# Nemo1999/Joint-TensoRF

Hardware: NVIDIA B200
Metric: rays/sec fwd+bwd (300^3 VM, 4096-ray batch) (higher is better)
Workload: dtype f32 (basis/shading GEMMs on tcgen05: bf16 operands, f32 accumulate)

## Files before the change

### include/jt_vm.h

```cpp
#ifndef JT_VM_H_
#define JT_VM_H_

#include <stdint.h>

#ifdef __cplusplus
extern "C" {
#endif

#ifndef __CUDA_RUNTIME_H__
typedef struct CUstream_st* cudaStream_t;
#endif

const char* jt_strerror(int code);
int jt_version(void);
long long jt_launch_count(void);

int jt_sample_ray_dense(const float* rays_o, const float* rays_d, const float* aux, int ndc, int n_rays,
                        int n_samples, const float* h_geom, const uint32_t* mask_bits, const int* h_mask_dims,
                        const float* h_mask_geom, float* pts, float* z, uint8_t* valid, cudaStream_t stream);

int jt_march_compact(const float* rays_o, const float* rays_d, const float* aux, int ndc, int n_rays,
                     int n_samples, const float* h_geom, const uint32_t* mask_bits, const int* h_mask_dims,
                     const float* h_mask_geom, int* ray_cnt, int* ray_off, int* sidx, float* samp, float* dist,
                     cudaStream_t stream);

int jt_exclusive_scan(const int* cnt, int* off, int n, cudaStream_t stream);

int jt_vm_gather_fwd(int app, const void* const* h_factors, const int* h_dims, const float* samp,
                     const int* slot, const int* n_dev, int n_max, float* out, cudaStream_t stream);

int jt_vm_gather_bwd(int app, const void* const* h_factors, void* const* h_factor_grads, const int* h_dims,
                     const float* samp, const int* slot, const int* n_dev, int n_max, const float* gin,
                     float* dsamp, int accumulate, cudaStream_t stream);

int jt_vm_scatter_rays(int app, const void* const* h_factors, void* const* h_factor_grads, const int* h_dims,
                       const float* samp, const int* slot, const int* sidx, const int* n_dev, int n_max,
                       const void* gin, int gin_bf16, int n_samples, const float* h_inv, float* d_o, float* d_d,
                       int max_ctas, int plane_mask, cudaStream_t stream);
int jt_ray_init(const float* rays_d, const float* dnorm, int n_rays, float* d_o, float* d_d, cudaStream_t stream);

int jt_gemm_nt(const float* X, int ldx, const float* W, int ldw, int w_kn, const float* bias, float* Y, int ldy,
               const float* mask, int ldm, const int* m_dev, int m_max, int N, int K, int act,
               cudaStream_t stream);
int jt_gemm_tn(const float* dY, int ldy, const float* X, int ldx, const int* m_dev, int m_max, int N, int K,
               float* dW, int ldw, float* db, cudaStream_t stream);
int jt_pe_encode(int bwd, int app_dim, int fea_pe, int view_pe, int mode, float fea_progress,
                 float view_progress, int n_samples, int normalize_dir, const float* feat, int ldf,
                 const int* aidx, const int* sidx, const float* rays_d, const int* n_dev, int n_max, float* out,
                 int ldo, float* out2, int ldo2, const float* din, int ldi, cudaStream_t stream);
int jt_sh_shade(int bwd, const float* feat, int ldf, const int* aidx, const int* sidx, const float* rays_d,
                int n_samples, int normalize_dir, const int* n_dev, int n_max, float* rgb, const float* dout,
                float* dfeat, int ldd, cudaStream_t stream);

int jt_tc_selftest(int mode, const float* A, int lda, const float* B, int ldb, float* D, int K, int N, int Ma,
                   cudaStream_t stream);
long long jt_head_tc_stage_bytes(int n_max);
int jt_head_fwd_tc(int split, const float* comps, const int* aidx, const int* sidx, const float* rays_d,
                   int n_samples, int normalize_dir, const float* Wb, const float* W1, const float* b1,
                   const float* W2, const float* b2, const float* W3, const float* b3, const int* n_dev, int n_max,
                   float fea_progress, float view_progress, float* rgb, float* feat_out, void* stage,
                   cudaStream_t stream);
int jt_app_basis_fwd_tc(int split, const void* const* h_factors, const int* h_dims, const float* samp,
                        const int* aidx, const int* sidx, const float* rays_d, int n_samples, int normalize_dir,
                        const float* Wb, const int* n_dev, int n_max, float* featdir, void* stage,
                        cudaStream_t stream);
int jt_head_mlp_fwd_tc(int split, const float* featdir, const float* W1, const float* b1, const float* W2,
                       const float* b2, const float* W3, const float* b3, const int* n_dev, int n_max,
                       float fea_progress, float view_progress, float* rgb, void* stage, cudaStream_t stream);
int jt_head_bwd_tc(const float* dout, const float* feat, int ldf, const float* Wb, const float* W1, const float* W2,
                   const float* W3, const int* n_dev, int n_max, float fea_progress, void* dcomps, int dcomps_bf16, void* stage,
                   float* gWb, float* gW1, float* gb1, float* gW2, float* gb2, float* gW3, float* gb3,
                   cudaStream_t stream);
int jt_app_basis_sh_fwd_tc(int split, const void* const* h_factors, const int* h_dims, const float* samp,
                           const int* aidx, const int* sidx, const float* rays_d, int n_samples, int normalize_dir,
                           const float* Wb, const int* n_dev, int n_max, float* featdir, float* rgb, void* stage,
                           cudaStream_t stream);
int jt_sh_bwd_tc(const float* dout, const float* featdir, int ldf, const float* Wb, const int* n_dev, int n_max,
                 void* dcomps, int dcomps_bf16, void* stage, float* gWb, cudaStream_t stream);

int jt_alpha_fwd(const int* ray_off, int n_rays, const float* sigfeat, const float* dist, const float* samp,
                 float density_shift, int act, float distance_scale, float thres, float* weight, float* trans,
                 float* acc, float* wz, int* app_cnt, int* app_off, int* aidx, int* app_of, int app_cap,
                 int* app_used, cudaStream_t stream);
int jt_composite_fwd(const int* app_off, int n_rays, const int* aidx, const float* weight, const float* rgb,
                     const float* acc, const float* wz, const float* rays_d, int white_bg, float depth_bias,
                     float* rgb_pre, float* rgb_map, float* depth, float* opacity, int app_cap, cudaStream_t stream);
int jt_render_bwd(const int* ray_off, int n_rays, const float* sigfeat, const float* dist, const float* weight,
                  const float* trans, const int* app_of, const float* rgb, const float* rgb_pre,
                  const float* g_rgb, const float* g_acc, float density_shift, int act, float distance_scale,
                  int white_bg, int shade_act, float* dout, float* dsig, float* dnorm, cudaStream_t stream);
int jt_blur_cl(const float* in, float* out, float* tmp, int H, int W, int C, const float* h_taps, int ntaps,
               int axes, int adjoint, cudaStream_t stream);
int jt_blur_multi(int n_arrays, const void* const* h_in, void* const* h_out, void* const* h_tmp, const int* h_dims,
                  const int* h_tapset, const float* h_taps, int nsets, int ntaps, int adjoint, cudaStream_t stream);

int jt_pose_rays_fwd(const float* se3, const int* view_idx, const float* base, int base_per_view,
                     const float* intr_inv, int kinv_per_view, const float* intr, int k_per_view, const int* pix,
                     int pix_per_view, int pix_base, int n_views, int n_rays_per_view, int width, int ndc,
                     int center_shift, int detach_shift, float near_plane, float* center, float* ray,
                     float* pose_out, cudaStream_t stream);
int jt_pose_rays_bwd(const float* se3, const int* view_idx, const float* base, int base_per_view,
                     const float* intr_inv, int kinv_per_view, const float* intr, int k_per_view, const int* pix,
                     int pix_per_view, int pix_base, int n_views, int n_rays_per_view, int width, int ndc,
                     int center_shift, int detach_shift, float near_plane, const float* d_center, const float* d_ray,
                     float* scratch12, float* d_se3, float* d_pose, cudaStream_t stream);

int jt_reg_values(int n_arrays, const void* const* h_x, const int* h_dims, const int* h_term, const int* h_l1,
                  double* sums_ws, float* out3, cudaStream_t stream);
int jt_reg_grads(int n_arrays, const void* const* h_x, void* const* h_g, const int* h_dims, const int* h_term,
                 const int* h_l1, const float* h_coef3, const float* up3, cudaStream_t stream);
int jt_adam_multi(int n_tensors, void* const* h_p, void* const* h_g, void* const* h_m, void* const* h_v,
                  const long long* h_numel, const double* h_lr, const int* h_step, double beta1, double beta2,
                  double eps, double grad_scale, int zero_grad, cudaStream_t stream);

int jt_field_alpha(const void* const* h_factors, const int* h_dims, const float* h_geom, const float* xyz,
                   long long n_points, const float* lin_x, const float* lin_y, const float* lin_z, const int* h_grid3,
                   const uint32_t* mask_bits, const int* h_mask_dims, const float* h_mask_geom, float density_shift,
                   int act, float length, float* alpha, cudaStream_t stream);
int jt_alpha_mask_build(const float* alpha, int W, int H, int D, float thres, float* tmp, float* vol, uint32_t* bits,
                        int* stats7, cudaStream_t stream);
int jt_resize_bilinear_cl(const float* in, int H, int W, int C, float* out, int H2, int W2, cudaStream_t stream);

int jt_image_blur(const float* in, float* out, float* tmp, int n_img, int H, int W, const float* h_taps, int ntaps,
                  cudaStream_t stream);
long long jt_edge_mask_ws_floats(int n_img, int H, int W);
int jt_edge_mask(const float* images, int n_img, int H, int W, int soft, float thresh, float* gg, float* ws,
                 float* stats, float* mask_f, uint8_t* mask_u8, cudaStream_t stream);
int jt_render_loss_fwd(const float* rgb, const float* images, const void* mask, int mask_kind, const int* ray_idx,
                       const int* view_idx, int n_views, int n_rays, int hw, int mode, float edge_factor,
                       float non_edge_factor, double* ws4, float* loss, cudaStream_t stream);
int jt_render_loss_bwd(const float* rgb, const float* images, const void* mask, int mask_kind, const int* ray_idx,
                       const int* view_idx, int n_views, int n_rays, int hw, int mode, float edge_factor,
                       float non_edge_factor, const double* ws4, const float* g_loss, float* d_rgb,
                       cudaStream_t stream);

long long jt_wv_stage_bytes(int n_max);
int jt_wv_head_fwd_tc(const float* comps, const int* aidx, const int* sidx, const float* rays_d, int n_samples,
                      int normalize_dir, const float* Wb, const float* W1, const float* b1, const float* W2,
                      const float* b2, const float* W3, const float* b3, const int* n_dev, int n_max,
                      float fea_progress, float view_progress, float* featdir, float* rgb, void* stage,
                      cudaStream_t stream);
int jt_wv_head_bwd_tc(const float* dout, const float* featdir, const float* Wb, const float* W1, const float* W2,
                      const float* W3, const int* n_dev, int n_max, float fea_progress, float* dcomps, void* stage,
                      float* gWb, float* gW1, float* gb1, float* gW2, float* gb2, float* gW3, float* gb3,
                      cudaStream_t stream);

int jt_cast_bf16_multi(int n_arrays, const void* const* h_src, void* const* h_dst, const long long* h_count,
                       cudaStream_t stream);

#ifdef __cplusplus
}
#endif
#endif
```

### joint-tensorf_b200/_lib.py

```python
import ctypes
import os

_HERE = os.path.dirname(os.path.abspath(__file__))
LIB_PATH = os.path.join(_HERE, "csrc", "libjt_vm.so")

_P, _I, _F, _D = ctypes.c_void_p, ctypes.c_int, ctypes.c_float, ctypes.c_double

SIGNATURES = {
    "jt_sample_ray_dense": [_P, _P, _P, _I, _I, _I, _P, _P, _P, _P, _P, _P, _P, _P],
    "jt_march_compact": [_P, _P, _P, _I, _I, _I, _P, _P, _P, _P, _P, _P, _P, _P, _P, _P],
    "jt_exclusive_scan": [_P, _P, _I, _P],
    "jt_vm_gather_fwd": [_I, _P, _P, _P, _P, _P, _I, _P, _P],
    "jt_vm_gather_bwd": [_I, _P, _P, _P, _P, _P, _P, _I, _P, _P, _I, _P],
    "jt_vm_scatter_rays": [_I, _P, _P, _P, _P, _P, _P, _P, _I, _P, _I, _I, _P, _P, _P, _I, _I, _P],
    "jt_ray_init": [_P, _P, _I, _P, _P, _P],
    "jt_gemm_nt": [_P, _I, _P, _I, _I, _P, _P, _I, _P, _I, _P, _I, _I, _I, _I, _P],
    "jt_gemm_tn": [_P, _I, _P, _I, _P, _I, _I, _I, _P, _I, _P, _P],
    "jt_pe_encode": [_I, _I, _I, _I, _I, _F, _F, _I, _I, _P, _I, _P, _P, _P, _P, _I, _P, _I, _P, _I, _P, _I, _P],
    "jt_sh_shade": [_I, _P, _I, _P, _P, _P, _I, _I, _P, _I, _P, _P, _P, _I, _P],
    "jt_tc_selftest": [_I, _P, _I, _P, _I, _P, _I, _I, _I, _P],
    "jt_head_fwd_tc": [_I, _P, _P, _P, _P, _I, _I, _P, _P, _P, _P, _P, _P, _P, _P, _I, _F, _F, _P, _P, _P, _P],
    "jt_app_basis_fwd_tc": [_I, _P, _P, _P, _P, _P, _P, _I, _I, _P, _P, _I, _P, _P, _P],
    "jt_head_mlp_fwd_tc": [_I, _P, _P, _P, _P, _P, _P, _P, _P, _I, _F, _F, _P, _P, _P],
    "jt_head_bwd_tc": [_P, _P, _I, _P, _P, _P, _P, _P, _I, _F, _P, _I, _P, _P, _P, _P, _P, _P, _P, _P, _P],
    "jt_app_basis_sh_fwd_tc": [_I, _P, _P, _P, _P, _P, _P, _I, _I, _P, _P, _I, _P, _P, _P, _P],
    "jt_sh_bwd_tc": [_P, _P, _I, _P, _P, _I, _P, _I, _P, _P, _P],
    "jt_alpha_fwd": [_P, _I, _P, _P, _P, _F, _I, _F, _F, _P, _P, _P, _P, _P, _P, _P, _P, _I, _P, _P],
    "jt_composite_fwd": [_P, _I, _P, _P, _P, _P, _P, _P, _I, _F, _P, _P, _P, _P, _I, _P],
    "jt_render_bwd": [_P, _I, _P, _P, _P, _P, _P, _P, _P, _P, _P, _F, _I, _F, _I, _I, _P, _P, _P, _P],
    "jt_blur_cl": [_P, _P, _P, _I, _I, _I, _P, _I, _I, _I, _P],
    "jt_blur_multi": [_I, _P, _P, _P, _P, _P, _P, _I, _I, _I, _P],
    "jt_pose_rays_fwd": [_P, _P, _P, _I, _P, _I, _P, _I, _P, _I, _I, _I, _I, _I, _I, _I, _I, _F, _P, _P, _P, _P],
    "jt_pose_rays_bwd": [_P, _P, _P, _I, _P, _I, _P, _I, _P, _I, _I, _I, _I, _I, _I, _I, _I, _F, _P, _P, _P, _P, _P, _P],
    "jt_reg_values": [_I, _P, _P, _P, _P, _P, _P, _P],
    "jt_reg_grads": [_I, _P, _P, _P, _P, _P, _P, _P, _P],
    "jt_field_alpha": [_P, _P, _P, _P, ctypes.c_longlong, _P, _P, _P, _P, _P, _P, _P, _F, _I, _F, _P, _P],
    "jt_alpha_mask_build": [_P, _I, _I, _I, _F, _P, _P, _P, _P, _P],
    "jt_resize_bilinear_cl": [_P, _I, _I, _I, _P, _I, _I, _P],
    "jt_image_blur": [_P, _P, _P, _I, _I, _I, _P, _I, _P],
    "jt_edge_mask": [_P, _I, _I, _I, _I, _F, _P, _P, _P, _P, _P, _P],
    "jt_render_loss_fwd": [_P, _P, _P, _I, _P, _P, _I, _I, _I, _I, _F, _F, _P, _P, _P],
    "jt_render_loss_bwd": [_P, _P, _P, _I, _P, _P, _I, _I, _I, _I, _F, _F, _P, _P, _P, _P],
    "jt_wv_head_fwd_tc": [_P, _P, _P, _P, _I, _I, _P, _P, _P, _P, _P, _P, _P, _P, _I, _F, _F, _P, _P, _P, _P],
    "jt_wv_head_bwd_tc": [_P, _P, _P, _P, _P, _P, _P, _I, _F, _P, _P, _P, _P, _P, _P, _P, _P, _P, _P],
    "jt_cast_bf16_multi": [_I, _P, _P, _P, _P],
    "jt_adam_multi": [_I, _P, _P, _P, _P, _P, _P, _P, _D, _D, _D, _D, _I, _P],
}

_lib = None


class JtError(RuntimeError):
    pass


def lib():
    global _lib
    if _lib is None:
        if not os.path.exists(LIB_PATH):
            raise JtError(
                f"{LIB_PATH} not found: the CUDA extension is not built. There is no CPU fallback; "
                "run `python -c \"import __graft_entry__ as g; g.build()\"`.")
        cdll = ctypes.CDLL(LIB_PATH)
        for name, args in SIGNATURES.items():
            fn = getattr(cdll, name)
            fn.argtypes = args
            fn.restype = _I
        cdll.jt_strerror.argtypes = [_I]
        cdll.jt_strerror.restype = ctypes.c_char_p
        cdll.jt_version.argtypes = []
        cdll.jt_version.restype = _I
        cdll.jt_head_tc_stage_bytes.argtypes = [_I]
        cdll.jt_head_tc_stage_bytes.restype = ctypes.c_longlong
        cdll.jt_wv_stage_bytes.argtypes = [_I]
        cdll.jt_wv_stage_bytes.restype = ctypes.c_longlong
        cdll.jt_edge_mask_ws_floats.argtypes = [_I, _I, _I]
        cdll.jt_edge_mask_ws_floats.restype = ctypes.c_longlong
        cdll.jt_launch_count.argtypes = []
        cdll.jt_launch_count.restype = ctypes.c_longlong
        _lib = cdll
    return _lib


def check(rc, what):
    if rc != 0:
        raise JtError(f"{what} failed: {lib().jt_strerror(rc).decode()} (code {rc})")


def launch_count():
    return int(lib().jt_launch_count())


def floats(vals):
    return (ctypes.c_float * len(vals))(*[float(v) for v in vals])


def ints(vals):
    return (ctypes.c_int * len(vals))(*[int(v) for v in vals])


def doubles(vals):
    return (ctypes.c_double * len(vals))(*[float(v) for v in vals])


def longlongs(vals):
    return (ctypes.c_longlong * len(vals))(*[int(v) for v in vals])


def ptrs(vals):
    return (ctypes.c_void_p * len(vals))(*[int(v) for v in vals])
```

### joint-tensorf_b200/csrc/shade_tc_bwd.cu

```cuda
#include "head_tc.cuh"
#include "../../include/jt_vm.h"

namespace jt {
using namespace tc;

struct BwdSmem {
    static constexpr int W2T = tile_bytes(H_, H_), W1T = tile_bytes(K1, H_), WBT = tile_bytes(CT, NB);
    static constexpr int off_w2t = 0, off_w1t = off_w2t + W2T, off_wbt = off_w1t + W1T;
    static constexpr int off_d2 = off_wbt + WBT, off_d1 = off_d2 + SZ_D2, off_df = off_d1 + SZ_D1, off_do = off_df + SZ_DF;
    static constexpr int off_w3 = off_do + SZ_DO;
    static constexpr int total = off_w3 + 3 * H_ * 4;
};

__device__ __forceinline__ uint32_t chunk_mask(const uint4 q) {
    const uint32_t w[4] = {q.x, q.y, q.z, q.w};
    uint32_t m = 0;
#pragma unroll
    for (int i = 0; i < 4; ++i) {
        m |= ((w[i] & 0x7FFFu) != 0u ? 1u : 0u) << (2 * i);
        m |= ((w[i] & 0x7FFF0000u) != 0u ? 1u : 0u) << (2 * i + 1);
    }
    return m;
}

constexpr int NTB = 2 * TM;

template <bool DC16>
__global__ void __launch_bounds__(NTB, 2) head_bwd_data_kernel(
    const float* __restrict__ dout, const float* __restrict__ feat_in, int ldf, const float* __restrict__ Wb,
    const float* __restrict__ W1, const float* __restrict__ W2, const float* __restrict__ W3,
    const int* __restrict__ n_dev, int n_fixed, float fprog, void* __restrict__ dcomps_out,
    unsigned char* __restrict__ stage) {
    using L = BwdSmem;
    extern __shared__ __align__(128) unsigned char smem[];
    __shared__ __align__(8) uint64_t bar;
    __shared__ uint32_t tmem_slot;
    const int tid = threadIdx.x, warp = tid >> 5;
    const int r = tid & (TM - 1), hh = tid >> 7;
    const int n = n_dev ? *n_dev : n_fixed;

    unsigned char* w2t = smem + L::off_w2t; unsigned char* w1t = smem + L::off_w1t; unsigned char* wbt = smem + L::off_wbt;
    unsigned char* D2 = smem + L::off_d2;   unsigned char* D1 = smem + L::off_d1;
    unsigned char* DF = smem + L::off_df;   unsigned char* DO = smem + L::off_do;
    float* w3s = reinterpret_cast<float*>(smem + L::off_w3);

    if (tid == 0) { mbar_init(&bar, 1); mbar_fence_init(); }
    if (warp == 0) tmem_alloc(&tmem_slot, 256);
    stage_tile(w2t, nullptr, H_, H_, [&](int i, int j) { return W2[(size_t)j * H_ + i]; });
    stage_tile(w1t, nullptr, K1, H_, [&](int c, int j) { const int rc = ref_col_l1(c); return rc >= 0 ? W1[(size_t)j * IN_ + rc] : 0.f; });
    stage_tile(wbt, nullptr, CT, NB, [&](int ic, int m) { return m < F_ ? Wb[(size_t)m * CT + ic] : 0.f; });
    for (int i = tid; i < 3 * H_; i += NTB) w3s[i] = W3[i];
    fence_async_smem();
    tc_fence_before();
    __syncthreads();
    tc_fence_after();
    const uint32_t tmem = tmem_slot;
    const uint32_t lane_addr = tmem + ((uint32_t)((warp & 3) * 32) << 16);
    const uint32_t T_DH1 = 0, T_DIN = 64, T_DC = 0;
    uint32_t phase = 0;
    const float pf0 = fminf(fmaxf(fprog * 2.f - 0.f, 0.f), 1.f), pf1 = fminf(fmaxf(fprog * 2.f - 1.f, 0.f), 1.f);

    float go[3];
    uint4 q3[4], q2[4];
    float feat[16];
    auto prefetch = [&](long long t) {
        const long long rw = t * TM + r;
        const bool lv = rw < n;
        const bool tv = t * TM < n;
        const unsigned char* stn = stage + (size_t)(tv ? t : 0) * STAGE_TILE_BYTES;
#pragma unroll
        for (int c4 = 0; c4 < 4; ++c4) {
            const size_t o = (size_t)(hh * 4 + c4) * TM * 16 + r * 16;
            q3[c4] = tv ? __ldg(reinterpret_cast<const uint4*>(stn + OFF_A3 + o)) : make_uint4(0, 0, 0, 0);
            q2[c4] = tv ? __ldg(reinterpret_cast<const uint4*>(stn + OFF_A2 + o)) : make_uint4(0, 0, 0, 0);
        }
        const float4* fp = reinterpret_cast<const float4*>(feat_in + (size_t)(lv ? rw : 0) * ldf) + 4 * hh;
#pragma unroll
        for (int q = 0; q < 4; ++q) {
            float4 f4 = make_float4(0.f, 0.f, 0.f, 0.f);
            if (lv && (hh == 0 || q < 3)) f4 = __ldg(fp + q);
            feat[4 * q] = f4.x; feat[4 * q + 1] = f4.y; feat[4 * q + 2] = f4.z; feat[4 * q + 3] = f4.w;
        }
        go[0] = go[1] = go[2] = 0.f;
        if (lv) {
            const float4 g4 = __ldg(reinterpret_cast<const float4*>(dout) + rw);
            go[0] = g4.x; go[1] = g4.y; go[2] = g4.z;
        }
    };
    prefetch(blockIdx.x);

    for (int tile = blockIdx.x; (long long)tile * TM < n; tile += gridDim.x) {
        const int row = tile * TM + r;
        const bool live = row < n;
        unsigned char* st = stage + (size_t)tile * STAGE_TILE_BYTES;
        if (hh == 0) {
            const float v[8] = {go[0], go[1], go[2], 0.f, 0.f, 0.f, 0.f, 0.f};
            store_chunk(DO, nullptr, TM, 0, r, v);
        }
#pragma unroll
        for (int c4 = 0; c4 < 4; ++c4) {
            const int c = hh * 4 + c4;
            const uint32_t m = chunk_mask(q3[c4]);
            float g[8];
#pragma unroll
            for (int i = 0; i < 8; ++i) {
                const int j = c * 8 + i;
                g[i] = ((m >> i) & 1u) ? go[0] * w3s[j] + go[1] * w3s[H_ + j] + go[2] * w3s[2 * H_ + j] : 0.f;
            }
            store_chunk(D2, nullptr, TM, c, r, g);
        }
        fence_async_smem();
        tc_fence_before();
        __syncthreads();
        if (tid == 0) {
            tc_fence_after();
            issue_gemm_kmajor<1>(tmem + T_DH1, D2, nullptr, w2t, nullptr, H_, H_, H_);
            mma_commit(&bar);
            bulk_s2g(st + OFF_D2, D2, SZ_D2);
            bulk_s2g(st + OFF_DO, DO, SZ_DO);
            bulk_commit();
        }
        mbar_wait(&bar, phase); phase ^= 1;
        tc_fence_after();
        {
            float g[32];
            tmem_ld32(lane_addr + T_DH1 + 32 * hh, g);
#pragma unroll
            for (int c = 0; c < 4; ++c) {
                const int cc = hh * 4 + c;
                const uint32_t m = chunk_mask(q2[c]);
                float v[8];
#pragma unroll
                for (int i = 0; i < 8; ++i) v[i] = ((m >> i) & 1u) ? g[c * 8 + i] : 0.f;
                store_chunk(D1, nullptr, TM, cc, r, v);
            }
        }
        fence_async_smem();
        tc_fence_before();
        __syncthreads();
        if (tid == 0) {
            tc_fence_after();
            issue_gemm_kmajor<1>(tmem + T_DIN, D1, nullptr, w1t, nullptr, H_, K1, K1);
            mma_commit(&bar);
            bulk_s2g(st + OFF_D1, D1, SZ_D1);
            bulk_commit();
        }
        mbar_wait(&bar, phase); phase ^= 1;
        tc_fence_after();
        {
            float df[16], raw[32];
            tmem_ld32(lane_addr + T_DIN, raw);
#pragma unroll
            for (int e = 0; e < 16; ++e) df[e] = (16 * hh + e < F_) ? (hh == 0 ? raw[e] : raw[16 + e]) : 0.f;
#pragma unroll
            for (int k = 0; k < 2; ++k) {
                float g[32];
                tmem_ld32(lane_addr + T_DIN + 32 + 64 * hh + 32 * k, g);
#pragma unroll
                for (int q = 0; q < 8; ++q) {
                    const int el = 8 * k + q;
                    if (16 * hh + el < F_) {
                        float sn, co;
                        fast_sincos(feat[el], &sn, &co);
                        const float s2 = 2.f * sn * co, c2 = 1.f - 2.f * sn * sn;
                        df[el] += pf0 * (co * g[4 * q] - sn * g[4 * q + 2]) + 2.f * pf1 * (c2 * g[4 * q + 1] - s2 * g[4 * q + 3]);
                    }
                }
            }
            store_chunk(DF, nullptr, TM, 2 * hh, r, df);
            store_chunk(DF, nullptr, TM, 2 * hh + 1, r, df + 8);
        }
        prefetch((long long)tile + gridDim.x);
        fence_async_smem();
        tc_fence_before();
        __syncthreads();
        if (tid == 0) {
            tc_fence_after();
            issue_gemm_kmajor<1>(tmem + T_DC, DF, nullptr, wbt, nullptr, NB, CT, CT);
            mma_commit(&bar);
            bulk_s2g(st + OFF_DF, DF, SZ_DF);
            bulk_commit();
        }
        mbar_wait(&bar, phase); phase ^= 1;
        tc_fence_after();
        store_dcomps_row<DC16>(lane_addr + T_DC, hh, live, row, dcomps_out);
        if (tid == 0) bulk_wait_read0();
        tc_fence_before();
        __syncthreads();
    }
    if (tid == 0) bulk_wait0();
    tc_fence_before();
    __syncthreads();
    if (warp == 0) tmem_dealloc(tmem, 256);
}

constexpr int WG_STAGES = 3;
constexpr int WG_A_REGION = 32768;
constexpr int WG_STAGE_BYTES = WG_A_REGION + SZ_A1;
constexpr int WG_SH_STAGES = 3;
constexpr int WG_SH_STAGE_BYTES = WG_A_REGION + SZ_A0;

struct WGroup { int a_off, a_bytes, b_off, b_bytes, n, col; };
__device__ __forceinline__ WGroup wgroup(int g) {
    switch (g) {
        case 0: return {OFF_D1, SZ_D1, OFF_A1, SZ_A1, K1, 0};
        case 1: return {OFF_D2, SZ_D2, OFF_A2, SZ_A2, K2, 160};
        case 2: return {OFF_DO, SZ_DO, OFF_A3, SZ_A3, K2, 240};
        default: return {OFF_DF, SZ_DF, OFF_A0, SZ_A0, CT, 320};
    }
}

template <int G0, int NG, int STAGES, int STAGE_BYTES>
__global__ void __launch_bounds__(TM) head_bwd_wgrad_kernel(const unsigned char* __restrict__ stage,
                                                            const int* __restrict__ n_dev, int n_fixed,
                                                            float* __restrict__ gWb, float* __restrict__ gW1,
                                                            float* __restrict__ gb1, float* __restrict__ gW2,
                                                            float* __restrict__ gb2, float* __restrict__ gW3,
                                                            float* __restrict__ gb3) {
    extern __shared__ __align__(128) unsigned char smem[];
    __shared__ __align__(8) uint64_t full[STAGES], empty[STAGES], done;
    __shared__ uint32_t tmem_slot;
    const int tid = threadIdx.x, warp = tid >> 5, lane = tid & 31;
    const int n = n_dev ? *n_dev : n_fixed;
    const int ntiles = (int)(((long long)n + TM - 1) / TM);
    const int my_tiles = blockIdx.x < ntiles ? (ntiles - 1 - blockIdx.x) / gridDim.x + 1 : 0;

    if (tid == 0) {
        for (int s = 0; s < STAGES; ++s) { mbar_init(&full[s], 1); mbar_init(&empty[s], 1); }
        mbar_init(&done, 1);
        mbar_fence_init();
    }
    if (warp == 0) tmem_alloc(&tmem_slot, 512);
    tc_fence_before();
    __syncthreads();
    tc_fence_after();
    const uint32_t tmem = tmem_slot;
    const int items = my_tiles * NG;

    if (warp == 0 && lane == 0) {
        for (int i = 0; i < items; ++i) {
            const int s = i % STAGES, round = i / STAGES;
            mbar_wait(&empty[s], (round & 1) ^ 1);
            const int tile = blockIdx.x + (i / NG) * gridDim.x;
            const WGroup g = wgroup(G0 + i % NG);
            const unsigned char* src = stage + (size_t)tile * STAGE_TILE_BYTES;
            unsigned char* dst = smem + s * STAGE_BYTES;
            mbar_expect_tx(&full[s], (uint32_t)(g.a_bytes + g.b_bytes));
            bulk_g2s(dst, src + g.a_off, g.a_bytes, &full[s]);
            bulk_g2s(dst + WG_A_REGION, src + g.b_off, g.b_bytes, &full[s]);
        }
    } else if (warp == 1 && lane == 0) {
        for (int i = 0; i < items; ++i) {
            const int s = i % STAGES, round = i / STAGES;
            mbar_wait(&full[s], round & 1);
            tc_fence_after();
            const WGroup g = wgroup(G0 + i % NG);
            const uint32_t a = smem_u32(smem + s * STAGE_BYTES), b = a + WG_A_REGION;
            const uint32_t idesc = idesc_bf16(128, g.n, 1, 1);
#pragma unroll
            for (int ks = 0; ks < TM / 16; ++ks)
                mma_bf16(tmem + g.col, smem_desc(a + ks * 256, 128, TM * 16), smem_desc(b + ks * 256, 128, TM * 16), idesc,
                         (i >= NG || ks > 0) ? 1u : 0u);
            mma_commit(&empty[s]);
        }
        mma_commit(&done);
    }
    __syncwarp();
    if (items > 0) {
        mbar_wait(&done, 0);
        tc_fence_after();
        if (warp < 2) {
            const uint32_t lane_addr = tmem + ((uint32_t)(warp * 32) << 16);
            const int m = tid;
            for (int c0 = 0; G0 == 0 && c0 < K1; c0 += 32) {
                float v[32];
                tmem_ld32(lane_addr + 0 + c0, v);
#pragma unroll
                for (int i = 0; i < 32; ++i) {
                    const int r = ref_col_l1(c0 + i);
                    if (r >= 0) atomicAdd(gW1 + (size_t)m * IN_ + r, v[i]);
                    else if (r == -2) atomicAdd(gb1 + m, v[i]);
                }
            }
            for (int c0 = 0; G0 == 0 && c0 < K2; c0 += 16) {
                float v[16], w[16];
                tmem_ld16(lane_addr + 160 + c0, v);
                tmem_ld16(lane_addr + 240 + c0, w);
#pragma unroll
                for (int i = 0; i < 16; ++i) {
                    const int c = c0 + i;
                    if (c < H_) { atomicAdd(gW2 + (size_t)m * H_ + c, v[i]); if (m < 3) atomicAdd(gW3 + (size_t)m * H_ + c, w[i]); }
                    else if (c == H_) { atomicAdd(gb2 + m, v[i]); if (m < 3) atomicAdd(gb3 + m, w[i]); }
                }
            }
            for (int c0 = 0; c0 < CT; c0 += 16) {
                float v[16];
                tmem_ld16(lane_addr + 320 + c0, v);
                if (m < F_) {
#pragma unroll
                    for (int i = 0; i < 16; ++i) atomicAdd(gWb + (size_t)m * CT + c0 + i, v[i]);
                }
            }
        }
    }
    tc_fence_before();
    __syncthreads();
    if (warp == 0) tmem_dealloc(tmem, 512);
}

struct ShBwdSmem {
    static constexpr int WBT = tile_bytes(CT, NB);
    static constexpr int OUT = TM * CT * 2;
    static constexpr int off_wbt = 0, off_df = off_wbt + WBT, off_out = off_df + 2 * SZ_DF;
    static constexpr int total = off_out + 2 * OUT;
};

__device__ __forceinline__ void bulk_wait_read_2() { asm volatile("cp.async.bulk.wait_group.read 2;" ::: "memory"); }

__global__ void __launch_bounds__(NTB, 2) sh_bwd_data_kernel(const float* __restrict__ dout, const float* __restrict__ featdir,
                                                             int ldf, const float* __restrict__ Wb,
                                                             const int* __restrict__ n_dev, int n_fixed,
                                                             unsigned short* __restrict__ dcomps_out,
                                                             unsigned char* __restrict__ stage) {
    using L = ShBwdSmem;
    extern __shared__ __align__(128) unsigned char smem[];
    __shared__ __align__(8) uint64_t bar;
    __shared__ uint32_t tmem_slot;
    const int tid = threadIdx.x, warp = tid >> 5;
    const int r = tid & (TM - 1), hh = tid >> 7;
    const int n = n_dev ? *n_dev : n_fixed;
    unsigned char* wbt = smem + L::off_wbt;

    if (tid == 0) { mbar_init(&bar, 1); mbar_fence_init(); }
    if (warp == 0) tmem_alloc(&tmem_slot, 256);
    stage_tile(wbt, nullptr, CT, NB, [&](int ic, int m) { return m < F_ ? Wb[(size_t)m * CT + ic] : 0.f; });
    fence_async_smem();
    tc_fence_before();
    __syncthreads();
    tc_fence_after();
    const uint32_t tmem = tmem_slot;
    const uint32_t lane_addr = tmem + ((uint32_t)((warp & 3) * 32) << 16);
    uint32_t phase = 0;
    int buf = 0;

    float4 g4, d4;
    auto prefetch = [&](long long t) {
        const long long rw = t * TM + r;
        g4 = d4 = make_float4(0.f, 0.f, 0.f, 0.f);
        if (rw < n) {
            g4 = __ldcs(reinterpret_cast<const float4*>(dout) + rw);
            d4 = __ldcs(reinterpret_cast<const float4*>(featdir + (size_t)rw * ldf + 28));
        }
    };
    prefetch(blockIdx.x);

    for (int tile = blockIdx.x; (long long)tile * TM < n; tile += gridDim.x, buf ^= 1) {
        const int rows = min(TM, n - tile * TM);
        unsigned char* st = stage + (size_t)tile * STAGE_TILE_BYTES;
        unsigned char* DF = smem + L::off_df + buf * SZ_DF;
        unsigned char* OUT = smem + L::off_out + buf * L::OUT;
        {
            const float d[3] = {d4.x, d4.y, d4.z};
            const float go[3] = {g4.x, g4.y, g4.z};
            float y[9], df[16];
            sh9(d, y);
#pragma unroll
            for (int e = 0; e < 16; ++e) {
                const int col = 16 * hh + e;
                const int c0 = e / 9, k0 = e % 9, c1 = (16 + e) / 9, k1 = (16 + e) % 9;
                const float v0 = go[c0] * y[k0];
                const float v1 = (16 + e) < F_ ? go[c1 < 3 ? c1 : 0] * y[k1] : 0.f;
                df[e] = col < F_ ? (hh == 0 ? v0 : v1) : 0.f;
            }
            store_chunk(DF, nullptr, TM, 2 * hh, r, df);
            store_chunk(DF, nullptr, TM, 2 * hh + 1, r, df + 8);
        }
        prefetch((long long)tile + gridDim.x);
        fence_async_smem();
        tc_fence_before();
        __syncthreads();
        if (tid == 0) {
            tc_fence_after();
            issue_gemm_kmajor<1>(tmem, DF, nullptr, wbt, nullptr, NB, CT, CT);
            bulk_s2g(st + OFF_DF, DF, SZ_DF);
            bulk_commit();
            bulk_wait_read_2();
            mma_commit(&bar);
        }
        mbar_wait(&bar, phase); phase ^= 1;
        tc_fence_after();
        {
            uint4* orow = reinterpret_cast<uint4*>(OUT + (size_t)r * (CT * 2));
#pragma unroll
            for (int k = 0; k < 2; ++k) {
                float g[32];
                const int c0 = 64 * hh + 32 * k;
                tmem_ld32(lane_addr + c0, g);
#pragma unroll
                for (int q = 0; q < 4; ++q)
                    orow[c0 / 8 + q] = make_uint4(pack_bf16(g[8 * q], g[8 * q + 1]), pack_bf16(g[8 * q + 2], g[8 * q + 3]),
                                                  pack_bf16(g[8 * q + 4], g[8 * q + 5]), pack_bf16(g[8 * q + 6], g[8 * q + 7]));
            }
            if (hh == 0) {
                float g[16];
                tmem_ld16(lane_addr + 128, g);
#pragma unroll
                for (int q = 0; q < 2; ++q)
                    orow[16 + q] = make_uint4(pack_bf16(g[8 * q], g[8 * q + 1]), pack_bf16(g[8 * q + 2], g[8 * q + 3]),
                                              pack_bf16(g[8 * q + 4], g[8 * q + 5]), pack_bf16(g[8 * q + 6], g[8 * q + 7]));
            }
        }
        fence_async_smem();
        tc_fence_before();
        __syncthreads();
        if (tid == 0) {
            bulk_s2g(dcomps_out + (size_t)tile * TM * CT, OUT, (uint32_t)rows * (CT * 2));
            bulk_commit();
        }
    }
    if (tid == 0) bulk_wait0();
    tc_fence_before();
    __syncthreads();
    if (warp == 0) tmem_dealloc(tmem, 256);
}

}

using namespace jt;

extern "C" long long jt_head_tc_stage_bytes(int n_max) {
    return (((long long)n_max + TM - 1) / TM) * STAGE_TILE_BYTES;
}

extern "C" int jt_head_bwd_tc(const float* dout, const float* feat, int ldf, const float* Wb, const float* W1, const float* W2,
                              const float* W3, const int* n_dev, int n_max, float fea_progress, void* dcomps,
                              int dcomps_bf16, void* stage, float* gWb, float* gW1, float* gb1, float* gW2, float* gb2, float* gW3,
                              float* gb3, cudaStream_t stream) {
    JT_CHECK_ARG(dout && feat && Wb && W1 && W2 && W3 && dcomps && stage && ldf >= 28 && ldf % 4 == 0);
    JT_CHECK_ARG(gWb && gW1 && gb1 && gW2 && gb2 && gW3 && gb3);
    JT_CHECK_ARG((reinterpret_cast<uintptr_t>(stage) & 127) == 0);
    if (n_max <= 0) return JT_OK;
    long long tiles = ((long long)n_max + TM - 1) / TM;
    int grid_d = (int)(tiles < 2 * kNumSMs ? tiles : 2 * kNumSMs);
    int grid_w = (int)(tiles < kNumSMs ? tiles : kNumSMs);
    if (int rc = set_smem(head_bwd_data_kernel<false>, BwdSmem::total)) return rc;
    if (int rc = set_smem(head_bwd_data_kernel<true>, BwdSmem::total)) return rc;
    if (int rc = set_smem(head_bwd_wgrad_kernel<0, 4, WG_STAGES, WG_STAGE_BYTES>, WG_STAGES * WG_STAGE_BYTES)) return rc;
    g_launches += 2;
    if (dcomps_bf16)
        head_bwd_data_kernel<true><<<grid_d, NTB, BwdSmem::total, stream>>>(dout, feat, ldf, Wb, W1, W2, W3, n_dev, n_max,
                                                                           fea_progress, dcomps, static_cast<unsigned char*>(stage));
    else
        head_bwd_data_kernel<false><<<grid_d, NTB, BwdSmem::total, stream>>>(dout, feat, ldf, Wb, W1, W2, W3, n_dev, n_max,
                                                                            fea_progress, dcomps, static_cast<unsigned char*>(stage));
    head_bwd_wgrad_kernel<0, 4, WG_STAGES, WG_STAGE_BYTES><<<grid_w, TM, WG_STAGES * WG_STAGE_BYTES, stream>>>(
        static_cast<const unsigned char*>(stage), n_dev, n_max, gWb, gW1, gb1, gW2, gb2, gW3, gb3);
    JT_RETURN_LAUNCH();
}

extern "C" int jt_sh_bwd_tc(const float* dout, const float* featdir, int ldf, const float* Wb, const int* n_dev,
                            int n_max, void* dcomps, int dcomps_bf16, void* stage, float* gWb, cudaStream_t stream) {
    JT_CHECK_ARG(dout && featdir && Wb && dcomps && stage && gWb && ldf >= 32 && ldf % 4 == 0);
    JT_CHECK_ARG(dcomps_bf16 == 1);
    JT_CHECK_ARG((reinterpret_cast<uintptr_t>(stage) & 127) == 0 && (reinterpret_cast<uintptr_t>(dcomps) & 15) == 0);
    if (n_max <= 0) return JT_OK;
    long long tiles = ((long long)n_max + TM - 1) / TM;
    int grid_d = (int)(tiles < 2 * kNumSMs ? tiles : 2 * kNumSMs);
    int grid_w = (int)(tiles < kNumSMs ? tiles : kNumSMs);
    if (int rc = set_smem(sh_bwd_data_kernel, ShBwdSmem::total)) return rc;
    if (int rc = set_smem(head_bwd_wgrad_kernel<3, 1, WG_SH_STAGES, WG_SH_STAGE_BYTES>, WG_SH_STAGES * WG_SH_STAGE_BYTES)) return rc;
    g_launches += 2;
    unsigned char* st = static_cast<unsigned char*>(stage);
    sh_bwd_data_kernel<<<grid_d, NTB, ShBwdSmem::total, stream>>>(dout, featdir, ldf, Wb, n_dev, n_max,
                                                                 static_cast<unsigned short*>(dcomps), st);
    head_bwd_wgrad_kernel<3, 1, WG_SH_STAGES, WG_SH_STAGE_BYTES><<<grid_w, TM, WG_SH_STAGES * WG_SH_STAGE_BYTES, stream>>>(
        st, n_dev, n_max, gWb, nullptr, nullptr, nullptr, nullptr, nullptr, nullptr);
    JT_RETURN_LAUNCH();
}
```

### joint-tensorf_b200/csrc/vm_scatter.cu

```cuda
#include <limits.h>
#include <stdlib.h>
#include <type_traits>
#include "jt_common.cuh"
#include "../../include/jt_vm.h"

namespace jt {

__device__ __forceinline__ float2 lo2(float4 v) { return make_float2(v.x, v.y); }
__device__ __forceinline__ float2 hi2(float4 v) { return make_float2(v.z, v.w); }
__device__ __forceinline__ float4 cat4(float2 l, float2 h) { return make_float4(l.x, l.y, h.x, h.y); }
__device__ __forceinline__ float2 dup2(float s) { return make_float2(s, s); }
__device__ __forceinline__ float4 f4z() { return make_float4(0.f, 0.f, 0.f, 0.f); }
__device__ __forceinline__ void f4_fma(float4& acc, float4 a, float2 s) {
    acc = cat4(__ffma2_rn(lo2(a), s, lo2(acc)), __ffma2_rn(hi2(a), s, hi2(acc)));
}
__device__ __forceinline__ float4 f4_mul2(float4 a, float4 b) { return cat4(__fmul2_rn(lo2(a), lo2(b)), __fmul2_rn(hi2(a), hi2(b))); }
__device__ __forceinline__ float4 f4_scale(float4 a, float2 s) { return cat4(__fmul2_rn(lo2(a), s), __fmul2_rn(hi2(a), s)); }
__device__ __forceinline__ void f2_dot_acc(float2& acc, float4 a, float4 b) {
    acc = __ffma2_rn(lo2(a), lo2(b), acc);
    acc = __ffma2_rn(hi2(a), hi2(b), acc);
}
__device__ __forceinline__ bool f4_any(float4 a) { return a.x != 0.f || a.y != 0.f || a.z != 0.f || a.w != 0.f; }

struct Pos { int i0; float f; float scale; };
__device__ __forceinline__ Pos axis_pos(float g, int n) {
    Pos p;
    p.scale = 0.5f * (float)(n - 1);
    const float x = (g + 1.0f) * p.scale;
    const float xf = floorf(x);
    p.f = x - xf;
    p.i0 = (int)fminf(fmaxf(xf, -2.0f), (float)n);
    return p;
}

struct ScatterArgs {
    Factors F;
    FactorGrads G;
    const float4* samp;
    const int* slot;
    const int* sidx;
    const int* n_dev;
    int n_fixed;
    const float* gin;
    int gin_bf16;
    float* d_o;
    float* d_d;
    float inv[3];
    int S;
    int seg;
    int seg_target;
    int plane_mask;
};

struct RaySums { float o[3], d[3]; };

constexpr int SC_THREADS = 128;

__device__ __forceinline__ void cp_async16(void* smem_dst, const void* gsrc) {
    asm volatile("cp.async.ca.shared.global [%0], [%1], 16;" ::"r"((uint32_t)__cvta_generic_to_shared(smem_dst)), "l"(gsrc) : "memory");
}
__device__ __forceinline__ void cp_async8(void* smem_dst, const void* gsrc) {
    asm volatile("cp.async.ca.shared.global [%0], [%1], 8;" ::"r"((uint32_t)__cvta_generic_to_shared(smem_dst)), "l"(gsrc) : "memory");
}
__device__ __forceinline__ void cp_async_commit() { asm volatile("cp.async.commit_group;" ::: "memory"); }
__device__ __forceinline__ void cp_async_wait1() { asm volatile("cp.async.wait_group 1;" ::: "memory"); }
__device__ __forceinline__ void cp_async_wait0() { asm volatile("cp.async.wait_group 0;" ::: "memory"); }

struct StepPos {
    int x0, y0, l0;
    float fx, fy, fl;
    float t;
    int sid;
};

template <bool APP, int NQ, int I, bool GB16, bool B16, int THR = SC_THREADS>
__device__ __forceinline__ void walk_plane(const ScatterArgs& A, const int e0, const int e1, const int q, const int qs,
                                           int& ray, int& ray_end, RaySums& rs,
                                           typename std::conditional<B16, uint2, float4>::type* __restrict__ sm) {
    using SlotT = typename std::conditional<B16, uint2, float4>::type;
    using ElemT = typename std::conditional<B16, unsigned short, float>::type;
    const Factors& F = A.F;
    constexpr int ax = I == 2 ? 1 : 0, ay = I == 0 ? 1 : 2, al = 2 - I;
    const int W = F.W[I], H = F.H[I], L = F.L[I], C = F.C[I];
    if (q >= C) return;
    const ElemT* __restrict__ P = reinterpret_cast<const ElemT*>(F.plane[I]) + q;
    const ElemT* __restrict__ Ln = reinterpret_cast<const ElemT*>(F.line[I]) + q;
    float* __restrict__ GP = A.G.plane[I] + q;
    float* __restrict__ GL = A.G.line[I] + q;
    const float sclx = 0.5f * (float)(W - 1), scly = 0.5f * (float)(H - 1), scll = 0.5f * (float)(L - 1);
    auto pslot = [&](int b, int c, int k) -> SlotT* { return sm + ((b * 4 + c) * NQ + k) * THR; };
    auto lslot = [&](int b, int c, int k) -> SlotT* { return sm + (8 * NQ + (b * 2 + c) * NQ + k) * THR; };
    auto rd = [&](const SlotT* p) -> float4 {
        if constexpr (B16) return bf16x4_to_f4(*p); else return *p;
    };
    auto cp = [&](SlotT* dst, const ElemT* src) { if constexpr (B16) cp_async8(dst, src); else cp_async16(dst, src); };

    auto make_pos = [&](const float4 u4, const int sid) {
        const float u[3] = {u4.x, u4.y, u4.z};
        StepPos p;
        const float fxp = (u[ax] + 1.0f) * sclx, fyp = (u[ay] + 1.0f) * scly, flp = (u[al] + 1.0f) * scll;
        const float xf = floorf(fxp), yf = floorf(fyp), lf = floorf(flp);
        p.x0 = (int)fminf(fmaxf(xf, -2.0f), (float)W); p.y0 = (int)fminf(fmaxf(yf, -2.0f), (float)H);
        p.l0 = (int)fminf(fmaxf(lf, -2.0f), (float)L);
        p.fx = fxp - xf; p.fy = fyp - yf; p.fl = flp - lf;
        p.t = u4.w; p.sid = sid;
        return p;
    };
    auto plane_offs = [&](int x0, int y0, unsigned o[4]) {
        const int xc0 = min(max(x0, 0), W - 1), xc1 = min(max(x0 + 1, 0), W - 1);
        const int yc0 = min(max(y0, 0), H - 1), yc1 = min(max(y0 + 1, 0), H - 1);
        o[0] = (unsigned)((yc0 * W + xc0) * C); o[1] = (unsigned)((yc0 * W + xc1) * C);
        o[2] = (unsigned)((yc1 * W + xc0) * C); o[3] = (unsigned)((yc1 * W + xc1) * C);
    };
    auto line_offs = [&](int l0, unsigned o[2]) {
        o[0] = (unsigned)(min(max(l0, 0), L - 1) * C); o[1] = (unsigned)(min(max(l0 + 1, 0), L - 1) * C);
    };
    auto fetch_plane = [&](int b, const unsigned o[4]) {
#pragma unroll
        for (int c = 0; c < 4; ++c)
#pragma unroll
            for (int k = 0; k < NQ; ++k) cp(pslot(b, c, k), P + o[c] + k * qs);
    };
    auto fetch_line = [&](int b, const unsigned o[2]) {
#pragma unroll
        for (int c = 0; c < 2; ++c)
#pragma unroll
            for (int k = 0; k < NQ; ++k) cp(lslot(b, c, k), Ln + o[c] + k * qs);
    };
    struct GinRaw { float4 f; uint2 h; float s; };
    auto load_gin = [&](int e, GinRaw g[NQ]) {
        if (APP && GB16) {
            const unsigned short* row = reinterpret_cast<const unsigned short*>(A.gin) + (size_t)e * F.ctot + F.off[I] + q;
#pragma unroll
            for (int k = 0; k < NQ; ++k) g[k].h = __ldcs(reinterpret_cast<const uint2*>(row + k * qs));
        } else if (APP) {
            const float* row = A.gin + (size_t)e * F.ctot + F.off[I] + q;
#pragma unroll
            for (int k = 0; k < NQ; ++k) g[k].f = __ldcs(reinterpret_cast<const float4*>(row + k * qs));
        } else {
            g[0].s = A.gin[e];
        }
    };
    auto gin_value = [&](const GinRaw g[NQ], int k) -> float4 {
        if (APP && GB16)
            return make_float4(__uint_as_float(g[k].h.x << 16), __uint_as_float(g[k].h.x & 0xFFFF0000u),
                               __uint_as_float(g[k].h.y << 16), __uint_as_float(g[k].h.y & 0xFFFF0000u));
        if (APP) return g[k].f;
        return make_float4(g[0].s, g[0].s, g[0].s, g[0].s);
    };

    int cx = INT_MIN, cy = INT_MIN, cl = INT_MIN;
    unsigned s00 = 0, s10 = 0, s01 = 0, s11 = 0, sl0 = 0, sl1 = 0;
    float4 g00[NQ], g10[NQ], g01[NQ], g11[NQ], gl0[NQ], gl1[NQ];
#pragma unroll
    for (int k = 0; k < NQ; ++k) { g00[k] = g10[k] = g01[k] = g11[k] = gl0[k] = gl1[k] = f4z(); }

    auto flush_ray = [&]() {
        if (ray >= 0) {
#pragma unroll
            for (int a = 0; a < 3; ++a) {
                if (rs.o[a] != 0.f) atomicAdd(A.d_o + 3 * ray + a, rs.o[a] * A.inv[a]);
                if (rs.d[a] != 0.f) atomicAdd(A.d_d + 3 * ray + a, rs.d[a] * A.inv[a]);
            }
        }
#pragma unroll
        for (int a = 0; a < 3; ++a) rs.o[a] = rs.d[a] = 0.f;
    };

    StepPos pn;
    unsigned on[4], oln[2];
    int pbn = 0, lbn = 0;
    {
        const int j0 = A.slot ? A.slot[e0] : e0;
        pn = make_pos(A.samp[j0], A.sidx[j0]);
        plane_offs(pn.x0, pn.y0, on);
        line_offs(pn.l0, oln);
        fetch_plane(0, on);
        fetch_line(0, oln);
        cp_async_commit();
    }
    auto slot_of = [&](int e) -> int { return e < e1 ? (A.slot ? A.slot[e] : e) : 0; };
    float4 un = f4z();
    int sn = 0;
    if (e0 + 1 < e1) {
        const int j1 = slot_of(e0 + 1);
        un = A.samp[j1];
        sn = A.sidx[j1];
    }
    int jn2 = slot_of(e0 + 2);
    GinRaw gn[NQ];
    load_gin(e0, gn);

    for (int e = e0; e < e1; ++e) {
        const StepPos pc = pn;
        const int pb = pbn, lb = lbn;
        const unsigned o00 = on[0], o10 = on[1], o01 = on[2], o11 = on[3], ol0 = oln[0], ol1 = oln[1];
        GinRaw gc[NQ];
#pragma unroll
        for (int k = 0; k < NQ; ++k) gc[k] = gn[k];
        if (e + 1 < e1) {
            pn = make_pos(un, sn);
            if (pn.x0 != pc.x0 || pn.y0 != pc.y0) {
                plane_offs(pn.x0, pn.y0, on);
                pbn = pb ^ 1;
                fetch_plane(pbn, on);
            }
            if (pn.l0 != pc.l0) {
                line_offs(pn.l0, oln);
                lbn = lb ^ 1;
                fetch_line(lbn, oln);
            }
            load_gin(e + 1, gn);
            if (e + 2 < e1) {
                un = A.samp[jn2];
                sn = A.sidx[jn2];
            }
            jn2 = slot_of(e + 3);
        }
        cp_async_commit();
        cp_async_wait1();

        if (pc.sid >= ray_end || pc.sid < ray_end - A.S) {
            flush_ray();
            ray = pc.sid / A.S;
            ray_end = (ray + 1) * A.S;
        }
        const int x0 = pc.x0, y0 = pc.y0, l0 = pc.l0;
        const float mx0 = (x0 >= 0 && x0 < W) ? 1.f : 0.f, mx1 = (x0 + 1 >= 0 && x0 + 1 < W) ? 1.f : 0.f;
        const float my0 = (y0 >= 0 && y0 < H) ? 1.f : 0.f, my1 = (y0 + 1 >= 0 && y0 + 1 < H) ? 1.f : 0.f;
        const float ml0 = (l0 >= 0 && l0 < L) ? 1.f : 0.f, ml1 = (l0 + 1 >= 0 && l0 + 1 < L) ? 1.f : 0.f;
        if (x0 != cx || y0 != cy) {
            if (cx != INT_MIN) {
#pragma unroll
                for (int k = 0; k < NQ; ++k) {
                    red_add_v4(GP + s00 + k * qs, g00[k]); red_add_v4(GP + s10 + k * qs, g10[k]);
                    red_add_v4(GP + s01 + k * qs, g01[k]); red_add_v4(GP + s11 + k * qs, g11[k]);
                }
            }
#pragma unroll
            for (int k = 0; k < NQ; ++k) { g00[k] = f4z(); g10[k] = f4z(); g01[k] = f4z(); g11[k] = f4z(); }
            cx = x0; cy = y0; s00 = o00; s10 = o10; s01 = o01; s11 = o11;
        }
        if (l0 != cl) {
            if (cl != INT_MIN) {
#pragma unroll
                for (int k = 0; k < NQ; ++k) { red_add_v4(GL + sl0 + k * qs, gl0[k]); red_add_v4(GL + sl1 + k * qs, gl1[k]); }
            }
#pragma unroll
            for (int k = 0; k < NQ; ++k) { gl0[k] = f4z(); gl1[k] = f4z(); }
            cl = l0; sl0 = ol0; sl1 = ol1;
        }
        const float fx = pc.fx, fy = pc.fy, fl = pc.fl;
        const float wx0 = (1.f - fx) * mx0, wx1 = fx * mx1, wy0 = (1.f - fy) * my0, wy1 = fy * my1;
        const float wl0 = (1.f - fl) * ml0, wl1 = fl * ml1;
        const float2 w00 = dup2(wx0 * wy0), w10 = dup2(wx1 * wy0), w01 = dup2(wx0 * wy1), w11 = dup2(wx1 * wy1);
        const float2 wl0p = dup2(wl0), wl1p = dup2(wl1);
        float2 dA2 = dup2(0.f), dB2 = dup2(0.f), dC2 = dup2(0.f), dD2 = dup2(0.f), dLa2 = dup2(0.f), dLb2 = dup2(0.f);
#pragma unroll
        for (int k = 0; k < NQ; ++k) {
            const float4 a = rd(pslot(pb, 0, k)), b = rd(pslot(pb, 1, k)), c = rd(pslot(pb, 2, k)), d = rd(pslot(pb, 3, k));
            const float4 la = rd(lslot(lb, 0, k)), lb4 = rd(lslot(lb, 1, k));
            float4 pv = f4_scale(a, w00), lv = f4_scale(la, wl0p);
            f4_fma(pv, b, w10); f4_fma(pv, c, w01); f4_fma(pv, d, w11);
            f4_fma(lv, lb4, wl1p);
            const float4 g4 = gin_value(gc, k);
            const float4 gl = f4_mul2(g4, lv);
            const float4 gp = f4_mul2(g4, pv);
            f4_fma(g00[k], gl, w00); f4_fma(g10[k], gl, w10); f4_fma(g01[k], gl, w01); f4_fma(g11[k], gl, w11);
            f4_fma(gl0[k], gp, wl0p); f4_fma(gl1[k], gp, wl1p);
            f2_dot_acc(dA2, gl, a); f2_dot_acc(dB2, gl, b); f2_dot_acc(dC2, gl, c); f2_dot_acc(dD2, gl, d);
            f2_dot_acc(dLa2, gp, la); f2_dot_acc(dLb2, gp, lb4);
        }
        const float dA = dA2.x + dA2.y, dB = dB2.x + dB2.y, dC = dC2.x + dC2.y, dD = dD2.x + dD2.y;
        const float dLa = dLa2.x + dLa2.y, dLb = dLb2.x + dLb2.y;
        const float dux = ((dB * mx1 - dA * mx0) * wy0 + (dD * mx1 - dC * mx0) * wy1) * sclx;
        const float duy = ((dC * my1 - dA * my0) * wx0 + (dD * my1 - dB * my0) * wx1) * scly;
        const float dul = (dLb * ml1 - dLa * ml0) * scll;
        const float t = pc.t;
        rs.o[ax] += dux; rs.d[ax] = fmaf(dux, t, rs.d[ax]);
        rs.o[ay] += duy; rs.d[ay] = fmaf(duy, t, rs.d[ay]);
        rs.o[al] += dul; rs.d[al] = fmaf(dul, t, rs.d[al]);
    }
    cp_async_wait0();
    if (cx != INT_MIN) {
#pragma unroll
        for (int k = 0; k < NQ; ++k) {
            red_add_v4(GP + s00 + k * qs, g00[k]); red_add_v4(GP + s10 + k * qs, g10[k]);
            red_add_v4(GP + s01 + k * qs, g01[k]); red_add_v4(GP + s11 + k * qs, g11[k]);
        }
    }
    if (cl != INT_MIN) {
#pragma unroll
        for (int k = 0; k < NQ; ++k) { red_add_v4(GL + sl0 + k * qs, gl0[k]); red_add_v4(GL + sl1 + k * qs, gl1[k]); }
    }
    flush_ray();
}

template <bool APP, int NQ, int MINB, bool GB16, int LWC, bool B16>
__global__ void __launch_bounds__(SC_THREADS, MINB) vm_scatter_walk_kernel(const ScatterArgs A, int LW_rt, int walkers_per_cta) {
    extern __shared__ __align__(16) unsigned char sc_smem[];
    using SlotT = typename std::conditional<B16, uint2, float4>::type;
    const int LW = LWC > 0 ? LWC : LW_rt;
    const int n = A.n_dev ? *A.n_dev : A.n_fixed;
    const int wl = threadIdx.x / LW;
    const int q = (threadIdx.x - wl * LW) * 4;
    const int qs = LW * 4;
    if (wl >= walkers_per_cta) return;
    SlotT* sm = reinterpret_cast<SlotT*>(sc_smem) + threadIdx.x;
    const int stride = gridDim.x * walkers_per_cta;
    int seg = A.seg;
    if (A.seg_target > 0) {
        const long long wt = (long long)stride * A.seg_target;
        const long long k = max(1LL, ((long long)n + wt / 2) / wt);
        seg = (int)max(1LL, ((long long)n + k * stride - 1) / (k * stride));
    }
    const int n_units = (n + seg - 1) / seg;
    for (int unit = blockIdx.x * walkers_per_cta + wl; unit < n_units; unit += stride) {
        const int e0 = unit * seg;
        const int e1 = min(e0 + seg, n);
        int ray = -1, ray_end = INT_MIN;
        RaySums rs;
#pragma unroll
        for (int a = 0; a < 3; ++a) rs.o[a] = rs.d[a] = 0.f;
        if (A.plane_mask & 1) walk_plane<APP, NQ, 0, GB16, B16>(A, e0, e1, q, qs, ray, ray_end, rs, sm);
        if (A.plane_mask & 2) walk_plane<APP, NQ, 1, GB16, B16>(A, e0, e1, q, qs, ray, ray_end, rs, sm);
        if (A.plane_mask & 4) walk_plane<APP, NQ, 2, GB16, B16>(A, e0, e1, q, qs, ray, ray_end, rs, sm);
    }
}

}

using namespace jt;

extern "C" int jt_vm_scatter_rays(int app, const void* const* h_factors, void* const* h_factor_grads,
                                  const int* h_dims, const float* samp, const int* slot, const int* sidx,
                                  const int* n_dev, int n_max, const void* gin, int gin_bf16, int n_samples, const float* h_inv,
                                  float* d_o, float* d_d, int max_ctas, int plane_mask, cudaStream_t stream) {
    JT_CHECK_ARG(h_factors && h_factor_grads && h_dims && samp && sidx && gin && h_inv && d_o && d_d && n_samples > 0);
    JT_CHECK_ARG(plane_mask > 0 && plane_mask <= 7);
    if (n_max <= 0) return JT_OK;
    ScatterArgs A;
    if (int rc = fill_factors(A.F, h_factors, h_dims)) return rc;
    int cmax = 0;
    for (int i = 0; i < 3; ++i) {
        A.G.plane[i] = static_cast<float*>(h_factor_grads[i]);
        A.G.line[i] = static_cast<float*>(h_factor_grads[3 + i]);
        JT_CHECK_ARG(A.G.plane[i] && A.G.line[i]);
        cmax = A.F.C[i] > cmax ? A.F.C[i] : cmax;
        JT_CHECK_ARG((long long)A.F.H[i] * A.F.W[i] * A.F.C[i] < 2147483647LL);
    }
    JT_CHECK_ARG((long long)n_max < 2147483647LL);
    A.samp = reinterpret_cast<const float4*>(samp);
    A.slot = slot; A.sidx = sidx; A.n_dev = n_dev; A.n_fixed = n_max; A.gin = static_cast<const float*>(gin); A.gin_bf16 = gin_bf16;
    JT_CHECK_ARG(!gin_bf16 || app);
    A.d_o = d_o; A.d_d = d_d;
    for (int a = 0; a < 3; ++a) A.inv[a] = h_inv[a];
    A.S = n_samples;
    A.plane_mask = plane_mask;
    static const int seg_env = getenv("JT_SCATTER_SEG") ? atoi(getenv("JT_SCATTER_SEG")) : 0;
    A.seg = seg_env > 0 ? seg_env : 32;
    A.seg_target = seg_env > 0 ? 0 : 100;
    if (max_ctas < 0) { A.seg = -max_ctas; A.seg_target = 0; max_ctas = 0; }
    int nq = 1, LW = cmax / 4;
    const bool uniform = A.F.C[0] == A.F.C[1] && A.F.C[1] == A.F.C[2];
    if (uniform && (cmax == 48 || cmax == 32)) { nq = cmax / 16; LW = 4; }
    JT_CHECK_ARG(LW >= 1 && LW <= 128);
    const int wpc = SC_THREADS / LW;
    const int threads = ((wpc * LW + 31) / 32) * 32;
    long long units = ((long long)n_max + A.seg - 1) / A.seg;
    long long want = (units + wpc - 1) / wpc;
    const int resident = nq == 3 ? 2 : (nq == 2 || app) ? 3 : 4;
    long long cap = max_ctas > 0 ? (long long)max_ctas
                                 : (A.seg_target > 0 ? (long long)kNumSMs * resident : (long long)kNumSMs * 32);
    if (A.seg_target > 0) want = cap;
    int grid = (int)(want < cap ? (want < 1 ? 1 : want) : cap);
    g_launches += 1;
    const int smem = 12 * nq * SC_THREADS * (A.F.bf16 ? 8 : 16);
#define JT_SCB(APPV, NQV, MB, GB, LWV, BV)                                                                          \
    {                                                                                                               \
        if (smem > 48 * 1024 &&                                                                                     \
            cudaFuncSetAttribute(vm_scatter_walk_kernel<APPV, NQV, MB, GB, LWV, BV>,                                \
                                 cudaFuncAttributeMaxDynamicSharedMemorySize, smem) != cudaSuccess)                 \
            return JT_ERR_LAUNCH;                                                                                   \
        vm_scatter_walk_kernel<APPV, NQV, MB, GB, LWV, BV><<<grid, threads, smem, stream>>>(A, LW, wpc);            \
    }
#define JT_SC(APPV, NQV, MB, GB, LWV) { if (A.F.bf16) JT_SCB(APPV, NQV, MB, GB, LWV, true) else JT_SCB(APPV, NQV, MB, GB, LWV, false) }
    if (app && gin_bf16) { if (nq == 3) JT_SC(true, 3, 2, true, 4) else if (nq == 2) JT_SC(true, 2, 3, true, 4) else JT_SC(true, 1, 3, true, 0) }
    else if (app) { if (nq == 3) JT_SC(true, 3, 2, false, 4) else if (nq == 2) JT_SC(true, 2, 3, false, 4) else JT_SC(true, 1, 3, false, 0) }
    else { if (nq == 3) JT_SC(false, 3, 2, false, 4) else if (nq == 2) JT_SC(false, 2, 3, false, 4) else JT_SC(false, 1, 4, false, 0) }
#undef JT_SC
#undef JT_SCB
    JT_RETURN_LAUNCH();
}
```

### joint-tensorf_b200/ops.py

```python
import contextlib

import torch

from . import _lib
from ._lib import check, floats, ints, longlongs, ptrs

MAT_MODE = ((0, 1), (0, 2), (1, 2))
VEC_MODE = (2, 1, 0)


class KernelTimer:

    def __init__(self):
        self.enabled = False
        self.records = []

    @contextlib.contextmanager
    def span(self, name):
        if not self.enabled:
            yield
            return
        s = torch.cuda.Event(enable_timing=True)
        e = torch.cuda.Event(enable_timing=True)
        s.record()
        yield
        e.record()
        self.records.append((name, s, e))

    def summary(self):
        torch.cuda.synchronize()
        out = {}
        for name, s, e in self.records:
            tot, cnt = out.get(name, (0.0, 0))
            out[name] = (tot + s.elapsed_time(e), cnt + 1)
        self.records = []
        return out


TIMER = KernelTimer()


def _stream():
    return torch.cuda.current_stream().cuda_stream


def _p(t):
    return 0 if t is None else t.data_ptr()


def _need_cuda(t, name):
    if not t.is_cuda:
        raise _lib.JtError(f"{name} must be a CUDA tensor: this path has no CPU implementation")


def phys_cl(x):
    assert x.dim() == 4 and x.shape[0] == 1, x.shape
    xp = x.permute(0, 2, 3, 1)
    if not xp.is_contiguous():
        xp = xp.contiguous()
    if xp.dtype != torch.float32:
        xp = xp.float()
    return xp[0]


class FactorSet:

    def __init__(self, planes, lines, store=None):
        self.planes = [phys_cl(p) for p in planes]
        self.lines = [phys_cl(l)[:, 0, :] for l in lines]
        self.C = [p.shape[2] for p in self.planes]
        for i in range(3):
            if self.C[i] % 4 != 0 or self.lines[i].shape[1] != self.C[i]:
                raise _lib.JtError(f"component count {self.C[i]} must be a multiple of 4 and match its line")
        self.store = store
        self.dims = ints([p.shape[0] for p in self.planes] + [p.shape[1] for p in self.planes] +
                         [l.shape[0] for l in self.lines] + self.C + [1 if store is not None else 0])
        src = store if store is not None else self.planes + self.lines
        self.ptrs = ptrs([t.data_ptr() for t in src])
        self.ctot = sum(self.C)

    def with_bf16_store(self, cache=None):
        srcs = self.planes + self.lines
        key = tuple((t.data_ptr(), t._version, tuple(t.shape)) for t in srcs)
        if cache is not None and cache.get("key") == key:
            store = cache["store"]
        else:
            store = [torch.empty(t.shape, device=t.device, dtype=torch.bfloat16) for t in srcs]
            cast_bf16_multi(srcs, store)
            if cache is not None:
                cache["key"], cache["store"] = key, store
        fs = FactorSet.__new__(FactorSet)
        fs.planes, fs.lines, fs.C, fs.ctot, fs.store = self.planes, self.lines, self.C, self.ctot, store
        fs.dims = ints(list(self.dims)[:12] + [1])
        fs.ptrs = ptrs([t.data_ptr() for t in store])
        return fs

    def zero_grads(self):
        gp = [torch.zeros_like(p) for p in self.planes]
        gl = [torch.zeros_like(l) for l in self.lines]
        return gp, gl

    @staticmethod
    def grads_as_nchw(gp, gl):
        return ([g.unsqueeze(0).permute(0, 3, 1, 2) for g in gp],
                [g.unsqueeze(0).unsqueeze(2).permute(0, 3, 1, 2) for g in gl])


def cast_bf16_multi(srcs, dsts):
    for a, b in zip(srcs, dsts):
        _need_cuda(a, "factor")
        assert a.is_contiguous() and b.is_contiguous() and a.dtype == torch.float32 and b.dtype == torch.bfloat16
    with TIMER.span("cast_bf16"):
        check(_lib.lib().jt_cast_bf16_multi(len(srcs), ptrs([a.data_ptr() for a in srcs]),
                                            ptrs([b.data_ptr() for b in dsts]), longlongs([a.numel() for a in srcs]),
                                            _stream()), "jt_cast_bf16_multi")


def sample_ray_dense(rays_o, rays_d, aux, ndc, n_samples, geom, mask=None):
    _need_cuda(rays_o, "rays_o")
    n = rays_o.shape[0]
    dev = rays_o.device
    pts = torch.empty((n, n_samples, 3), device=dev)
    z = torch.empty((n, n_samples), device=dev)
    valid = torch.empty((n, n_samples), device=dev, dtype=torch.uint8)
    mb, md, mg = (mask.bits, mask.h_dims, mask.h_geom) if mask is not None else (None, None, None)
    with TIMER.span("sample_ray_dense"):
        check(_lib.lib().jt_sample_ray_dense(_p(rays_o), _p(rays_d), _p(aux), int(ndc), n, n_samples, geom,
                                             _p(mb), md, mg, _p(pts), _p(z), _p(valid), _stream()),
              "jt_sample_ray_dense")
    return pts, z, valid.bool()


class Compacted:
    __slots__ = ("n_rays", "n_samples", "cap", "ray_off", "sidx", "samp", "dist", "count")


def march_compact(rays_o, rays_d, aux, ndc, n_samples, geom, mask=None):
    _need_cuda(rays_o, "rays_o")
    n = rays_o.shape[0]
    dev = rays_o.device
    cap = max(n * n_samples, 1)
    c = Compacted()
    c.n_rays, c.n_samples, c.cap = n, n_samples, cap
    ray_cnt = torch.empty((max(n, 1),), device=dev, dtype=torch.int32)
    c.ray_off = torch.zeros((n + 1,), device=dev, dtype=torch.int32)
    c.sidx = torch.empty((cap,), device=dev, dtype=torch.int32)
    c.samp = torch.empty((cap, 4), device=dev)
    c.dist = torch.empty((cap,), device=dev)
    mb, md, mg = (mask.bits, mask.h_dims, mask.h_geom) if mask is not None else (None, None, None)
    with TIMER.span("march_compact"):
        check(_lib.lib().jt_march_compact(_p(rays_o), _p(rays_d), _p(aux), int(ndc), n, n_samples, geom,
                                          _p(mb), md, mg, _p(ray_cnt), _p(c.ray_off), _p(c.sidx), _p(c.samp),
                                          _p(c.dist), _stream()), "jt_march_compact")
    c.count = c.ray_off[n:n + 1]
    return c


def vm_gather_fwd(app, fs, samp, slot, n_dev, n_max, out):
    with TIMER.span("vm_app_fwd" if app else "vm_density_fwd"):
        check(_lib.lib().jt_vm_gather_fwd(int(app), fs.ptrs, fs.dims, _p(samp), _p(slot), _p(n_dev), int(n_max),
                                          _p(out), _stream()), "jt_vm_gather_fwd")


def vm_gather_bwd(app, fs, gp, gl, samp, slot, n_dev, n_max, gin, dsamp, accumulate):
    gptrs = ptrs([g.data_ptr() for g in gp] + [g.data_ptr() for g in gl])
    with TIMER.span("vm_app_bwd" if app else "vm_density_bwd"):
        check(_lib.lib().jt_vm_gather_bwd(int(app), fs.ptrs, gptrs, fs.dims, _p(samp), _p(slot), _p(n_dev),
                                          int(n_max), _p(gin), _p(dsamp), int(accumulate), _stream()),
              "jt_vm_gather_bwd")


def vm_scatter_rays(app, fs, gp, gl, samp, slot, sidx, n_dev, n_max, gin, n_samples, h_inv, d_o, d_d, max_ctas=0,
                    plane_mask=7):
    gptrs = ptrs([g.data_ptr() for g in gp] + [g.data_ptr() for g in gl])
    with TIMER.span("vm_app_bwd" if app else "vm_density_bwd"):
        check(_lib.lib().jt_vm_scatter_rays(int(app), fs.ptrs, gptrs, fs.dims, _p(samp), _p(slot), _p(sidx),
                                            _p(n_dev), int(n_max), _p(gin), int(gin.dtype == torch.bfloat16),
                                            int(n_samples), h_inv, _p(d_o), _p(d_d), int(max_ctas), int(plane_mask),
                                            _stream()),
              "jt_vm_scatter_rays")


def gemm_nt(x, ldx, w, ldw, w_kn, bias, y, ldy, mask, ldm, m_dev, m_max, n, k, act, name="gemm_nt",
            x_off=0, w_off=0, y_off=0, mask_off=0):
    with TIMER.span(name):
        check(_lib.lib().jt_gemm_nt(_p(x) + 4 * x_off, ldx, _p(w) + 4 * w_off, ldw, int(w_kn), _p(bias),
                                    _p(y) + 4 * y_off, ldy, (_p(mask) + 4 * mask_off) if mask is not None else 0,
                                    ldm, _p(m_dev), int(m_max), n, k, act, _stream()), "jt_gemm_nt")


def gemm_tn(dy, ldy, x, ldx, m_dev, m_max, n, k, dw, ldw, db, name="gemm_tn", dy_off=0, x_off=0, dw_off=0):
    with TIMER.span(name):
        check(_lib.lib().jt_gemm_tn(_p(dy) + 4 * dy_off, ldy, _p(x) + 4 * x_off, ldx, _p(m_dev), int(m_max), n, k,
                                    _p(dw) + 4 * dw_off, ldw, _p(db), _stream()), "jt_gemm_tn")


def pe_encode(bwd, app_dim, fea_pe, view_pe, mode, fprog, vprog, n_samples, normalize_dir, feat, ldf, aidx, sidx,
              rays_d, n_dev, n_max, out, ldo, out2=None, ldo2=0, din=None, ldi=0):
    with TIMER.span("pe_bwd" if bwd else "pe_fwd"):
        check(_lib.lib().jt_pe_encode(int(bwd), app_dim, fea_pe, view_pe, mode, float(fprog), float(vprog),
                                      n_samples, int(normalize_dir), _p(feat), ldf, _p(aidx), _p(sidx), _p(rays_d),
                                      _p(n_dev), int(n_max), _p(out), ldo, _p(out2), ldo2, _p(din), ldi, _stream()),
              "jt_pe_encode")


def sh_shade(bwd, feat, ldf, aidx, sidx, rays_d, n_samples, normalize_dir, n_dev, n_max, rgb, dout, dfeat, ldd):
    with TIMER.span("sh_bwd" if bwd else "sh_fwd"):
        check(_lib.lib().jt_sh_shade(int(bwd), _p(feat), ldf, _p(aidx), _p(sidx), _p(rays_d), n_samples,
                                     int(normalize_dir), _p(n_dev), int(n_max), _p(rgb), _p(dout), _p(dfeat), ldd,
                                     _stream()), "jt_sh_shade")


def tc_selftest(mode, a, b, k, n, ma=0):
    d = torch.zeros((128, n), device=a.device)
    check(_lib.lib().jt_tc_selftest(mode, _p(a), a.shape[1], _p(b), b.shape[1], _p(d), k, n, ma, _stream()),
          "jt_tc_selftest")
    return d


def head_tc_stage(n_max, device):
    nbytes = int(_lib.lib().jt_head_tc_stage_bytes(int(n_max)))
    return torch.empty((nbytes,), device=device, dtype=torch.uint8)


def head_fwd_tc(split, comps, aidx, sidx, rays_d, n_samples, normalize_dir, wb, w1, b1, w2, b2, w3, b3, n_dev, n_max,
                fprog, vprog, rgb, feat_out=None, stage=None):
    with TIMER.span("head_fwd_tc"):
        check(_lib.lib().jt_head_fwd_tc(split, _p(comps), _p(aidx), _p(sidx), _p(rays_d), n_samples,
                                        int(normalize_dir), _p(wb), _p(w1), _p(b1), _p(w2), _p(b2), _p(w3), _p(b3),
                                        _p(n_dev), int(n_max), float(fprog), float(vprog), _p(rgb), _p(feat_out),
                                        _p(stage), _stream()), "jt_head_fwd_tc")


def app_basis_fwd_tc(split, fs, samp, aidx, sidx, rays_d, n_samples, normalize_dir, wb, n_dev, n_max, featdir,
                     stage=None):
    with TIMER.span("app_basis_fwd_tc"):
        check(_lib.lib().jt_app_basis_fwd_tc(split, fs.ptrs, fs.dims, _p(samp), _p(aidx), _p(sidx), _p(rays_d),
                                             int(n_samples), int(normalize_dir), _p(wb), _p(n_dev), int(n_max),
                                             _p(featdir), _p(stage), _stream()), "jt_app_basis_fwd_tc")


def app_basis_sh_fwd_tc(split, fs, samp, aidx, sidx, rays_d, n_samples, normalize_dir, wb, n_dev, n_max, featdir, rgb,
                        stage=None):
    with TIMER.span("app_basis_sh_fwd_tc"):
        check(_lib.lib().jt_app_basis_sh_fwd_tc(split, fs.ptrs, fs.dims, _p(samp), _p(aidx), _p(sidx), _p(rays_d),
                                                int(n_samples), int(normalize_dir), _p(wb), _p(n_dev), int(n_max),
                                                _p(featdir), _p(rgb), _p(stage), _stream()), "jt_app_basis_sh_fwd_tc")


def sh_bwd_tc(dout, featdir, wb, n_dev, n_max, dcomps, stage, g_basis):
    with TIMER.span("sh_bwd_tc"):
        check(_lib.lib().jt_sh_bwd_tc(_p(dout), _p(featdir), int(featdir.shape[1]), _p(wb), _p(n_dev), int(n_max),
                                      _p(dcomps), int(dcomps.dtype == torch.bfloat16), _p(stage), _p(g_basis),
                                      _stream()), "jt_sh_bwd_tc")


def head_mlp_fwd_tc(split, featdir, w1, b1, w2, b2, w3, b3, n_dev, n_max, fprog, vprog, rgb, stage=None):
    with TIMER.span("head_mlp_fwd_tc"):
        check(_lib.lib().jt_head_mlp_fwd_tc(split, _p(featdir), _p(w1), _p(b1), _p(w2), _p(b2), _p(w3), _p(b3),
                                            _p(n_dev), int(n_max), float(fprog), float(vprog), _p(rgb), _p(stage),
                                            _stream()), "jt_head_mlp_fwd_tc")


def head_bwd_tc(dout, feat, wb, w1, w2, w3, n_dev, n_max, fprog, dcomps, stage, grads):
    with TIMER.span("head_bwd_tc"):
        check(_lib.lib().jt_head_bwd_tc(_p(dout), _p(feat), int(feat.shape[1]), _p(wb), _p(w1), _p(w2), _p(w3), _p(n_dev), int(n_max),
                                        float(fprog), _p(dcomps), int(dcomps.dtype == torch.bfloat16), _p(stage),
                                        *[_p(g) for g in grads], _stream()),
              "jt_head_bwd_tc")


def wv_stage(n_max, device):
    nbytes = int(_lib.lib().jt_wv_stage_bytes(int(n_max)))
    return torch.empty((nbytes,), device=device, dtype=torch.uint8)


def wv_head_fwd_tc(comps, aidx, sidx, rays_d, n_samples, normalize_dir, wb, w1, b1, w2, b2, w3, b3, n_dev, n_max, fprog,
                   vprog, featdir, rgb, stage=None):
    with TIMER.span("wv_head_fwd_tc"):
        check(_lib.lib().jt_wv_head_fwd_tc(_p(comps), _p(aidx), _p(sidx), _p(rays_d), int(n_samples), int(normalize_dir),
                                           _p(wb), _p(w1), _p(b1), _p(w2), _p(b2), _p(w3), _p(b3), _p(n_dev), int(n_max),
                                           float(fprog), float(vprog), _p(featdir), _p(rgb), _p(stage), _stream()),
              "jt_wv_head_fwd_tc")


def wv_head_bwd_tc(dout, featdir, wb, w1, w2, w3, n_dev, n_max, fprog, dcomps, stage, grads):
    with TIMER.span("wv_head_bwd_tc"):
        check(_lib.lib().jt_wv_head_bwd_tc(_p(dout), _p(featdir), _p(wb), _p(w1), _p(w2), _p(w3), _p(n_dev), int(n_max),
                                           float(fprog), _p(dcomps), _p(stage), *[_p(g) for g in grads], _stream()),
              "jt_wv_head_bwd_tc")


def host_taps(kernel):
    if isinstance(kernel, (list, tuple)):
        vals = list(kernel)
    else:
        vals = getattr(kernel, "_jt_host", None)
        if vals is None:
            vals = kernel.detach().reshape(-1).float().cpu().tolist()
    return floats(vals), len(vals)


def blur_cl(x_phys, h, w, c, taps, axes, adjoint):
    out = torch.empty_like(x_phys)
    tmp = torch.empty_like(x_phys) if axes == 3 else None
    h_taps, ntaps = taps
    with TIMER.span("blur_adj" if adjoint else "blur_fwd"):
        check(_lib.lib().jt_blur_cl(_p(x_phys), _p(out), _p(tmp), h, w, c, h_taps, ntaps, axes,
                                    int(adjoint), _stream()), "jt_blur_cl")
    return out


def blur_multi(arrays, metas, tapsets, adjoint):
    outs = [torch.empty_like(a) for a in arrays]
    tmps = [torch.empty_like(a) if m[3] == 3 else None for a, m in zip(arrays, metas)]
    ntaps = len(tapsets[0])
    assert all(len(t) == ntaps for t in tapsets)
    flat = floats([v for t in tapsets for v in t])
    dims = ints([v for m in metas for v in m[:4]])
    sets = ints([m[4] for m in metas])
    with TIMER.span("blur_adj" if adjoint else "blur_fwd"):
        check(_lib.lib().jt_blur_multi(len(arrays), ptrs([a.data_ptr() for a in arrays]),
                                       ptrs([o.data_ptr() for o in outs]), ptrs([_p(t) for t in tmps]), dims, sets,
                                       flat, len(tapsets), ntaps, int(adjoint), _stream()), "jt_blur_multi")
    return outs


class BlurGroup(torch.autograd.Function):

    @staticmethod
    def forward(ctx, metas, tapsets, *factors):
        xs, full = [], []
        for x, (hq, wq, axes, ts) in zip(factors, metas):
            _need_cuda(x, "factor")
            xp = phys_cl(x)
            c = xp.shape[2]
            assert xp.shape[0] * xp.shape[1] == hq * wq
            xs.append(xp)
            full.append((hq, wq, c, axes, ts))
        ys = blur_multi(xs, full, tapsets, 0)
        ctx.meta = (full, tapsets, [tuple(xp.shape) for xp in xs])
        return tuple(y.view(1, m[0], m[1], m[2]).permute(0, 3, 1, 2) for y, m in zip(ys, full))

    @staticmethod
    def backward(ctx, *gys):
        full, tapsets, shapes = ctx.meta
        idx = [i for i, g in enumerate(gys) if g is not None and ctx.needs_input_grad[2 + i]]
        gxs = blur_multi([phys_cl(gys[i]) for i in idx], [full[i] for i in idx], tapsets, 1) if idx else []
        out = [None] * len(gys)
        for i, gx in zip(idx, gxs):
            out[i] = gx.view(1, *shapes[i]).permute(0, 3, 1, 2)
        return (None, None, *out)


class BlurFactor(torch.autograd.Function):

    @staticmethod
    def forward(ctx, x, taps, hq, wq, axes):
        _need_cuda(x, "factor")
        xp = phys_cl(x)
        c = xp.shape[2]
        assert xp.shape[0] * xp.shape[1] == hq * wq
        ht = host_taps(taps)
        y = blur_cl(xp, hq, wq, c, ht, axes, 0)
        ctx.meta = (tuple(xp.shape), hq, wq, c, axes, ht)
        return y.view(1, hq, wq, c).permute(0, 3, 1, 2)

    @staticmethod
    def backward(ctx, gy):
        shape, hq, wq, c, axes, ht = ctx.meta
        gp = phys_cl(gy)
        gx = blur_cl(gp, hq, wq, c, ht, axes, 1)
        return gx.view(1, *shape).permute(0, 3, 1, 2), None, None, None, None


def _samp_from_xyz(xyz_norm):
    n = xyz_norm.shape[0]
    samp = torch.zeros((max(n, 1), 4), device=xyz_norm.device)
    samp[:n, :3] = xyz_norm.detach()
    return samp


class DensityFeature(torch.autograd.Function):

    @staticmethod
    def forward(ctx, xyz, *factors):
        _need_cuda(xyz, "xyz_sampled")
        fs = FactorSet(factors[:3], factors[3:])
        n = xyz.shape[0]
        samp = _samp_from_xyz(xyz)
        out = torch.empty((max(n, 1),), device=xyz.device)
        vm_gather_fwd(0, fs, samp, None, None, n, out)
        ctx.fs, ctx.samp, ctx.n = fs, samp, n
        return out[:n]

    @staticmethod
    def backward(ctx, g):
        fs, samp, n = ctx.fs, ctx.samp, ctx.n
        gp, gl = fs.zero_grads()
        dsamp = torch.zeros_like(samp)
        vm_gather_bwd(0, fs, gp, gl, samp, None, None, n, g.contiguous().float(), dsamp, 0)
        gpn, gln = FactorSet.grads_as_nchw(gp, gl)
        return (dsamp[:n, :3], *gpn, *gln)


class AppComponents(torch.autograd.Function):

    @staticmethod
    def forward(ctx, xyz, *factors):
        _need_cuda(xyz, "xyz_sampled")
        fs = FactorSet(factors[:3], factors[3:])
        n = xyz.shape[0]
        samp = _samp_from_xyz(xyz)
        out = torch.empty((max(n, 1), fs.ctot), device=xyz.device)
        vm_gather_fwd(1, fs, samp, None, None, n, out)
        ctx.fs, ctx.samp, ctx.n = fs, samp, n
        return out[:n]

    @staticmethod
    def backward(ctx, g):
        fs, samp, n = ctx.fs, ctx.samp, ctx.n
        gp, gl = fs.zero_grads()
        dsamp = torch.zeros_like(samp)
        vm_gather_bwd(1, fs, gp, gl, samp, None, None, n, g.contiguous().float(), dsamp, 0)
        gpn, gln = FactorSet.grads_as_nchw(gp, gl)
        return (dsamp[:n, :3], *gpn, *gln)


class Linear(torch.autograd.Function):

    @staticmethod
    def forward(ctx, x, w, b):
        m, k = x.shape
        n = w.shape[0]
        ldx, ldy = (k + 3) & ~3, (n + 3) & ~3
        xp = x if (ldx == k and x.is_contiguous()) else torch.nn.functional.pad(x, (0, ldx - k)).contiguous()
        y = torch.empty((max(m, 1), ldy), device=x.device)
        wc = w.contiguous()
        gemm_nt(xp, ldx, wc, k, 0, b, y, ldy, None, 0, None, m, n, k, 0, name="basis_fwd")
        ctx.save_for_backward(xp, wc)
        ctx.meta = (m, n, k, ldx, ldy, b is not None)
        return y[:m, :n]

    @staticmethod
    def backward(ctx, gy):
        xp, wc = ctx.saved_tensors
        m, n, k, ldx, ldy, has_b = ctx.meta
        g = torch.zeros((max(m, 1), ldy), device=gy.device)
        g[:m, :n] = gy
        gx = torch.empty((max(m, 1), ldx), device=gy.device)
        gemm_nt(g, ldy, wc, k, 1, None, gx, ldx, None, 0, None, m, k, n, 0, name="basis_bwd_x")
        gw = torch.zeros_like(wc)
        gb = torch.zeros((n,), device=gy.device) if has_b else None
        gemm_tn(g, ldy, xp, ldx, None, m, n, k, gw, k, gb, name="basis_bwd_w")
        return gx[:m, :k], gw, gb


def field_alpha(fs, geom, shift, act, length, xyz=None, lin=None, grid=None, mask=None):
    mb, md, mg = (mask.bits, mask.h_dims, mask.h_geom) if mask is not None else (None, None, None)
    if xyz is not None:
        _need_cuda(xyz, "xyz")
        xyz = xyz.reshape(-1, 3).contiguous().float()
        n = xyz.shape[0]
        out = torch.empty((n,), device=xyz.device)
        lx = ly = lz = None
        g3 = None
    else:
        lx, ly, lz = lin
        _need_cuda(lx, "linspace table")
        n = 0
        out = torch.empty((grid[2], grid[1], grid[0]), device=lx.device)
        g3 = ints(grid)
    with TIMER.span("field_alpha"):
        check(_lib.lib().jt_field_alpha(fs.ptrs, fs.dims, geom, _p(xyz), n, _p(lx), _p(ly), _p(lz), g3, _p(mb), md, mg,
                                        float(shift), int(act), float(length), _p(out), _stream()), "jt_field_alpha")
    return out


def alpha_mask_build(alpha_zyx, thres):
    _need_cuda(alpha_zyx, "alpha")
    assert alpha_zyx.is_contiguous() and alpha_zyx.dtype == torch.float32
    d, h, w = alpha_zyx.shape
    dev = alpha_zyx.device
    tmp = torch.empty_like(alpha_zyx)
    vol = torch.empty_like(alpha_zyx)
    bits = torch.empty(((d * h * w + 31) // 32,), device=dev, dtype=torch.int32)
    stats = torch.empty((7,), device=dev, dtype=torch.int32)
    with TIMER.span("alpha_mask_build"):
        check(_lib.lib().jt_alpha_mask_build(_p(alpha_zyx), w, h, d, float(thres), _p(tmp), _p(vol), _p(bits),
                                             _p(stats), _stream()), "jt_alpha_mask_build")
    return vol, bits, stats


def resize_bilinear_cl(x, h2, w2):
    _need_cuda(x, "factor")
    xp = phys_cl(x)
    h, w, c = xp.shape
    out = torch.empty((h2, w2, c), device=x.device, dtype=torch.float32)
    with TIMER.span("resize_bilinear"):
        check(_lib.lib().jt_resize_bilinear_cl(_p(xp), h, w, c, _p(out), int(h2), int(w2), _stream()),
              "jt_resize_bilinear_cl")
    return out.unsqueeze(0).permute(0, 3, 1, 2)
```

### joint-tensorf_b200/render.py

```python
import torch

from . import _lib, ops
from ._lib import check, floats
from .ops import FactorSet, TIMER, _p, _stream


def _r4(n):
    return (n + 3) & ~3


class RenderCfg:

    def __init__(self, **kw):
        self.n_samples = 0
        self.ndc = False
        self.white_bg = True
        self.h_geom = None
        self.h_inv = None
        self.mask = None
        self.density_shift = -10.0
        self.act = 0
        self.distance_scale = 25.0
        self.thres = 1e-4
        self.depth_bias = 0.0
        self.shading = "MLP_Fea"
        self.app_dim = 27
        self.fea_pe = 2
        self.view_pe = 2
        self.hidden = 64
        self.fea_prog = 1.0
        self.view_prog = 1.0
        self.head = "fp32"
        self.tc_fwd_split = 2
        self.grad_enabled = True
        self.tc_infer_fp16 = True
        self.storage = "fp32"
        self.store_cache = (None, None)
        self.bf16_backward_taps = False
        self.app_cap = None
        self.app_monitor = None
        self.infer_exact_alloc = True
        self.__dict__.update(kw)


def tc_supported(cfg, afs=None, raise_if_not=False, comps=None):
    comps = list(afs.C) if afs is not None else (list(comps) if comps is not None else None)
    c48 = comps is None or all(int(c) == 48 for c in comps)
    ok = (cfg.shading == "MLP_Fea" and cfg.app_dim == 27 and cfg.hidden == 64 and cfg.fea_pe == 2 and
          cfg.view_pe == 2 and c48)
    ok = ok or (cfg.shading == "SH" and cfg.app_dim == 27 and c48)
    c20 = comps is None or all(int(c) == 20 for c in comps)
    ok = ok or (cfg.shading == "MLP_Fea_WeakView" and cfg.app_dim == 20 and cfg.hidden == 32 and cfg.fea_pe == 2 and
                cfg.view_pe == 2 and c20)
    if not ok and raise_if_not:
        raise _lib.JtError("head='tc' needs 3 x 48 appearance components, app_dim 27 and MLP_Fea (hidden 64, pe 2) or "
                           "SH shading, or 3 x 20 components, app_dim 20 and MLP_Fea_WeakView (hidden 32, pe 2); "
                           "use head='fp32'")
    return ok


class _Head:

    @staticmethod
    def forward(cfg, ws, feat, ldf, aidx, sidx, rays_d, a_count, cap, params, dev):
        F, H = cfg.app_dim, cfg.hidden
        rgb = torch.empty((cap, 4), device=dev)
        if cfg.shading == "SH":
            ops.sh_shade(0, feat, ldf, aidx, sidx, rays_d, cfg.n_samples, cfg.ndc, a_count, cap, rgb, None, None, 0)
            return rgb
        w1, b1, w2, b2, w3, b3 = params
        if cfg.shading == "MLP_Fea":
            in_dim = F + 3 + 2 * cfg.fea_pe * F + 6 * cfg.view_pe
            ldi = _r4(in_dim)
            x = torch.empty((cap, ldi), device=dev)
            ops.pe_encode(0, F, cfg.fea_pe, cfg.view_pe, 0, cfg.fea_prog, cfg.view_prog, cfg.n_samples, cfg.ndc,
                          feat, ldf, aidx, sidx, rays_d, a_count, cap, x, ldi)
            h1 = torch.empty((cap, H), device=dev)
            ops.gemm_nt(x, ldi, w1, in_dim, 0, b1, h1, H, None, 0, a_count, cap, H, in_dim, 1, name="mlp_l1_fwd")
            h2 = torch.empty((cap, H), device=dev)
            ops.gemm_nt(h1, H, w2, H, 0, b2, h2, H, None, 0, a_count, cap, H, H, 1, name="mlp_l2_fwd")
            ops.gemm_nt(h2, H, w3, H, 0, b3, rgb, 4, None, 0, a_count, cap, 3, H, 2, name="mlp_l3_fwd")
            ws.update(x=x, ldi=ldi, in_dim=in_dim, h1=h1, h2=h2)
        elif cfg.shading == "MLP_Fea_WeakView":
            in_dim = F + 2 * cfg.fea_pe * F
            ldi = _r4(in_dim)
            nv = 6 * cfg.view_pe
            assert nv % 4 == 0, "view_pe must be even for the WeakView layout"
            ldm = nv + H
            x = torch.empty((cap, ldi), device=dev)
            mid = torch.empty((cap, ldm), device=dev)
            ops.pe_encode(0, F, cfg.fea_pe, cfg.view_pe, 1, cfg.fea_prog, cfg.view_prog, cfg.n_samples, cfg.ndc,
                          feat, ldf, aidx, sidx, rays_d, a_count, cap, x, ldi, mid, ldm)
            h1 = torch.empty((cap, H), device=dev)
            ops.gemm_nt(x, ldi, w1, in_dim, 0, b1, h1, H, None, 0, a_count, cap, H, in_dim, 1, name="mlp_l1_fwd")
            ops.gemm_nt(h1, H, w2, H, 0, b2, mid, ldm, None, 0, a_count, cap, H, H, 1, name="mlp_l2_fwd", y_off=nv)
            ops.gemm_nt(mid, ldm, w3, ldm, 0, b3, rgb, 4, None, 0, a_count, cap, 3, ldm, 2, name="mlp_l3_fwd")
            ws.update(x=x, ldi=ldi, in_dim=in_dim, h1=h1, mid=mid, ldm=ldm, nv=nv)
        else:
            raise _lib.JtError(f"shading model {cfg.shading!r} is not implemented by the B200 path")
        return rgb

    @staticmethod
    def backward(cfg, ws, dout, feat, ldf, aidx, sidx, rays_d, a_count, cap, params, dev):
        F, H = cfg.app_dim, cfg.hidden
        dfeat = torch.empty((cap, ldf), device=dev)
        if cfg.shading == "SH":
            ops.sh_shade(1, feat, ldf, aidx, sidx, rays_d, cfg.n_samples, cfg.ndc, a_count, cap, None, dout, dfeat, ldf)
            return dfeat, []
        w1, b1, w2, b2, w3, b3 = params
        gw1, gb1, gw2, gb2, gw3, gb3 = [torch.zeros_like(t) for t in params]
        x, ldi, in_dim, h1 = ws["x"], ws["ldi"], ws["in_dim"], ws["h1"]
        dh2 = torch.empty((cap, H), device=dev)
        dh1 = torch.empty((cap, H), device=dev)
        if cfg.shading == "MLP_Fea":
            h2 = ws["h2"]
            ops.gemm_tn(dout, 4, h2, H, a_count, cap, 3, H, gw3, H, gb3, name="mlp_l3_bwd_w")
            ops.gemm_nt(dout, 4, w3, H, 1, None, dh2, H, h2, H, a_count, cap, H, 3, 0, name="mlp_l3_bwd_x")
        else:
            mid, ldm, nv = ws["mid"], ws["ldm"], ws["nv"]
            ops.gemm_tn(dout, 4, mid, ldm, a_count, cap, 3, ldm, gw3, ldm, gb3, name="mlp_l3_bwd_w")
            ops.gemm_nt(dout, 4, w3, ldm, 1, None, dh2, H, mid, ldm, a_count, cap, H, 3, 0, name="mlp_l3_bwd_x",
                        w_off=nv, mask_off=nv)
        ops.gemm_tn(dh2, H, h1, H, a_count, cap, H, H, gw2, H, gb2, name="mlp_l2_bwd_w")
        ops.gemm_nt(dh2, H, w2, H, 1, None, dh1, H, h1, H, a_count, cap, H, H, 0, name="mlp_l2_bwd_x")
        ops.gemm_tn(dh1, H, x, ldi, a_count, cap, H, in_dim, gw1, in_dim, gb1, name="mlp_l1_bwd_w")
        ops.gemm_nt(dh1, H, w1, in_dim, 1, None, x, ldi, None, 0, a_count, cap, in_dim, H, 0, name="mlp_l1_bwd_x")
        mode = 0 if cfg.shading == "MLP_Fea" else 1
        ops.pe_encode(1, F, cfg.fea_pe, cfg.view_pe, mode, cfg.fea_prog, cfg.view_prog, cfg.n_samples, cfg.ndc,
                      feat, ldf, None, None, None, a_count, cap, dfeat, ldf, None, 0, x, ldi)
        return dfeat, [gw1, gb1, gw2, gb2, gw3, gb3]


class VMRender(torch.autograd.Function):

    @staticmethod
    def forward(ctx, cfg, rays_o, rays_d, aux, *tensors):
        ops._need_cuda(rays_o, "rays_o")
        lib = _lib.lib()
        dev = rays_o.device
        rays_o = rays_o.detach().contiguous().float()
        rays_d = rays_d.detach().contiguous().float()
        dens, app, basis_w, head = tensors[0:6], tensors[6:12], tensors[12], tensors[13:]
        head = [t.detach().contiguous() for t in head]
        basis_w = basis_w.detach().contiguous()
        dfs = FactorSet([t.detach() for t in dens[:3]], [t.detach() for t in dens[3:]])
        afs = FactorSet([t.detach() for t in app[:3]], [t.detach() for t in app[3:]])
        dfs32, afs32 = dfs, afs
        if cfg.storage == "bf16":
            dfs = dfs.with_bf16_store(cfg.store_cache[0])
            afs = afs.with_bf16_store(cfg.store_cache[1])
            if cfg.bf16_backward_taps:
                dfs32, afs32 = dfs, afs
        N, S = rays_o.shape[0], cfg.n_samples
        F = cfg.app_dim
        ldf = _r4(F)
        if basis_w.shape != (F, afs.ctot):
            raise _lib.JtError(f"basis_mat weight {tuple(basis_w.shape)} != ({F}, {afs.ctot})")

        comp = ops.march_compact(rays_o, rays_d, aux, cfg.ndc, S, cfg.h_geom, cfg.mask)
        cap = comp.cap
        sigfeat = torch.empty((cap,), device=dev)
        ops.vm_gather_fwd(0, dfs, comp.samp, None, comp.count, cap, sigfeat)

        weight = torch.empty((cap,), device=dev)
        trans = torch.empty((cap,), device=dev)
        acc = torch.empty((N,), device=dev)
        wz = torch.empty((N,), device=dev)
        app_cnt = torch.empty((N,), device=dev, dtype=torch.int32)
        app_off = torch.zeros((N + 1,), device=dev, dtype=torch.int32)
        aidx = torch.empty((cap,), device=dev, dtype=torch.int32)
        app_of = torch.empty((cap,), device=dev, dtype=torch.int32)
        train = cfg.grad_enabled and any(ctx.needs_input_grad)
        acap = cap if (cfg.app_cap is None or not train) else max(1, min(cap, int(cfg.app_cap)))
        app_used = torch.zeros((2,), device=dev, dtype=torch.int32)
        with TIMER.span("alpha_fwd"):
            check(lib.jt_alpha_fwd(_p(comp.ray_off), N, _p(sigfeat), _p(comp.dist), _p(comp.samp),
                                   float(cfg.density_shift), cfg.act, float(cfg.distance_scale), float(cfg.thres),
                                   _p(weight), _p(trans), _p(acc), _p(wz), _p(app_cnt), _p(app_off), _p(aidx),
                                   _p(app_of), int(acap), _p(app_used), _stream()), "jt_alpha_fwd")
        a_count = app_used[0:1]
        if not train and cfg.infer_exact_alloc:
            acap = max(int(a_count.item()), 1)
        cap_v, cap = cap, acap

        ws = {}
        comps = None
        if cfg.head == "tc" and cfg.shading == "MLP_Fea_WeakView":
            tc_supported(cfg, afs, raise_if_not=True)
            comps = torch.empty((cap, afs.ctot), device=dev)
            ops.vm_gather_fwd(1, afs, comp.samp, aidx, a_count, cap, comps)
            feat = torch.empty((cap, 32), device=dev)
            rgb = torch.empty((cap, 4), device=dev)
            ws["stage"] = ops.wv_stage(cap, dev) if train else None
            ops.wv_head_fwd_tc(comps, aidx, comp.sidx, rays_d, S, cfg.ndc, basis_w, *head, a_count, cap, cfg.fea_prog,
                               cfg.view_prog, feat, rgb, ws["stage"])
            comps = None
        elif cfg.head == "tc":
            tc_supported(cfg, afs, raise_if_not=True)
            rgb = torch.empty((cap, 4), device=dev)
            feat = torch.empty((cap, 32), device=dev)
            ws["stage"] = ops.head_tc_stage(cap, dev) if train else None
            if cfg.shading == "SH":
                ops.app_basis_sh_fwd_tc(cfg.tc_fwd_split, afs, comp.samp, aidx, comp.sidx, rays_d, S, cfg.ndc,
                                        basis_w, a_count, cap, feat, rgb, ws["stage"])
            else:
                ops.app_basis_fwd_tc(cfg.tc_fwd_split, afs, comp.samp, aidx, comp.sidx, rays_d, S, cfg.ndc, basis_w,
                                     a_count, cap, feat, ws["stage"])
                mlp_split = 3 if (not train and cfg.tc_infer_fp16 and cfg.tc_fwd_split == 2) else cfg.tc_fwd_split
                ops.head_mlp_fwd_tc(mlp_split, feat, *head, a_count, cap, cfg.fea_prog, cfg.view_prog, rgb,
                                    ws["stage"])
        else:
            comps = torch.empty((cap, afs.ctot), device=dev)
            ops.vm_gather_fwd(1, afs, comp.samp, aidx, a_count, cap, comps)
            feat = torch.empty((cap, ldf), device=dev)
            ops.gemm_nt(comps, afs.ctot, basis_w, afs.ctot, 0, None, feat, ldf, None, 0, a_count, cap, F, afs.ctot, 0,
                        name="basis_fwd")
            rgb = _Head.forward(cfg, ws, feat, ldf, aidx, comp.sidx, rays_d, a_count, cap, head, dev)

        rgb_pre = torch.empty((N, 3), device=dev)
        rgb_map = torch.empty((N, 3), device=dev)
        depth = torch.empty((N,), device=dev)
        opacity = torch.empty((N,), device=dev)
        with TIMER.span("composite_fwd"):
            check(lib.jt_composite_fwd(_p(app_off), N, _p(aidx), _p(weight), _p(rgb), _p(acc), _p(wz), _p(rays_d),
                                       int(cfg.white_bg), float(cfg.depth_bias), _p(rgb_pre), _p(rgb_map),
                                       _p(depth), _p(opacity), int(cap), _stream()), "jt_composite_fwd")

        ctx.cfg, ctx.comp, ctx.dfs, ctx.afs, ctx.ws = cfg, comp, dfs32, afs32, ws
        ctx.bufs = dict(rays_d=rays_d, sigfeat=sigfeat, weight=weight, trans=trans, app_off=app_off, aidx=aidx,
                        app_of=app_of, comps=comps, feat=feat, rgb=rgb, rgb_pre=rgb_pre, basis_w=basis_w, head=head,
                        a_count=a_count)
        ctx.n_head = len(head)
        ctx.acap = cap
        ctx.save_for_backward(*tensors)
        ctx.mark_non_differentiable(depth)
        VMRender.last_counts = (comp.count, app_off[N:N + 1])
        VMRender.last_app_used = app_used
        if cfg.app_monitor is not None and train:
            cfg.app_monitor(app_off[N:N + 1], app_used, N)
        return rgb_map, depth, opacity

    @staticmethod
    def backward(ctx, g_rgb, g_depth, g_acc):
        lib = _lib.lib()
        cfg, comp, dfs, afs, ws, b = ctx.cfg, ctx.comp, ctx.dfs, ctx.afs, ctx.ws, ctx.bufs
        _ = ctx.saved_tensors
        if ws.get("consumed"):
            raise _lib.JtError("second backward through the same render call: the strict-fp32 MLP head reuses its "
                               "encoded-input buffer for the input gradient (2.6 GB at 4096 x 1000 samples); call "
                               "forward again, or use head_precision='tc' / SH shading, whose backward is re-entrant")
        dev = g_rgb.device
        N, cap_v, cap = comp.n_rays, comp.cap, ctx.acap
        F = cfg.app_dim
        ldf = _r4(F)
        g_rgb = g_rgb.contiguous().float()
        g_acc = g_acc.contiguous().float() if g_acc is not None else None
        shade_act = 2 if cfg.shading == "SH" else 1

        dout = torch.empty((cap, 4), device=dev)
        dsig = torch.empty((cap_v,), device=dev)
        dnorm = torch.empty((N,), device=dev) if cfg.ndc else None
        with TIMER.span("render_bwd"):
            check(lib.jt_render_bwd(_p(comp.ray_off), N, _p(b["sigfeat"]), _p(comp.dist), _p(b["weight"]),
                                    _p(b["trans"]), _p(b["app_of"]), _p(b["rgb"]), _p(b["rgb_pre"]), _p(g_rgb),
                                    _p(g_acc), float(cfg.density_shift), cfg.act, float(cfg.distance_scale),
                                    int(cfg.white_bg), shade_act, _p(dout), _p(dsig), _p(dnorm), _stream()),
                  "jt_render_bwd")

        if VMRender.debug_capture is not None:
            VMRender.debug_capture.update(dsig=dsig.clone(), dout=dout.clone(), count=comp.count.clone(),
                                          weight=b["weight"].clone(), trans=b["trans"].clone(), rgb=b["rgb"].clone(),
                                          sigfeat=b["sigfeat"].clone(), a_count=b["a_count"].clone())

        sync = getattr(cfg, "grad_sync", None)
        if sync is not None and not sync._active():
            sync = None
        shapes = [p.shape for p in afs.planes] + [l.shape for l in afs.lines] + \
                 [p.shape for p in dfs.planes] + [l.shape for l in dfs.lines] + \
                 [b["basis_w"].shape] + [t.shape for t in b["head"]]
        sizes = [int(torch.Size(s).numel()) for s in shapes]
        flat = torch.zeros((sum(sizes),), device=dev)
        views, o = [], 0
        for s, n in zip(shapes, sizes):
            views.append(flat[o:o + n].view(s))
            o += n
        gap, gal, gdp, gdl = views[0:3], views[3:6], views[6:9], views[9:12]
        g_basis, head_grads = views[12], views[13:]
        n_app = sum(sizes[0:6])

        d_o = torch.empty((N, 3), device=dev)
        d_d = torch.empty((N, 3), device=dev)
        with TIMER.span("ray_init"):
            check(lib.jt_ray_init(_p(b["rays_d"]), _p(dnorm), N, _p(d_o), _p(d_d), _stream()), "jt_ray_init")

        wv_tc = cfg.head == "tc" and cfg.shading == "MLP_Fea_WeakView"
        dcomps = torch.empty((cap, afs.ctot), device=dev,
                             dtype=torch.bfloat16 if (cfg.head == "tc" and not wv_tc) else torch.float32)
        if wv_tc:
            w1, b1, w2, b2, w3, b3 = b["head"]
            ops.wv_head_bwd_tc(dout, b["feat"], b["basis_w"], w1, w2, w3, b["a_count"], cap, cfg.fea_prog, dcomps,
                               ws["stage"], (g_basis, *head_grads))
        elif cfg.head == "tc" and cfg.shading == "SH":
            ops.sh_bwd_tc(dout, b["feat"], b["basis_w"], b["a_count"], cap, dcomps, ws["stage"], g_basis)
        elif cfg.head == "tc":
            w1, b1, w2, b2, w3, b3 = b["head"]
            ops.head_bwd_tc(dout, b["feat"], b["basis_w"], w1, w2, w3, b["a_count"], cap, cfg.fea_prog, dcomps,
                            ws["stage"], (g_basis, *head_grads))
        else:
            dfeat, hg = _Head.backward(cfg, ws, dout, b["feat"], ldf, b["aidx"], comp.sidx, b["rays_d"],
                                       b["a_count"], cap, b["head"], dev)
            if cfg.shading != "SH":
                ws["consumed"] = True
            for dst, src in zip(head_grads, hg):
                dst.copy_(src)
            ops.gemm_tn(dfeat, ldf, b["comps"], afs.ctot, b["a_count"], cap, F, afs.ctot, g_basis, afs.ctot, None,
                        name="basis_bwd_w")
            ops.gemm_nt(dfeat, ldf, b["basis_w"], afs.ctot, 1, None, dcomps, afs.ctot, None, 0, b["a_count"], cap,
                        afs.ctot, F, 0, name="basis_bwd_x")
        if sync is None:
            ops.vm_scatter_rays(1, afs, gap, gal, comp.samp, b["aidx"], comp.sidx, b["a_count"], cap, dcomps,
                                cfg.n_samples, cfg.h_inv, d_o, d_d)
            ops.vm_scatter_rays(0, dfs, gdp, gdl, comp.samp, None, comp.sidx, comp.count, cap_v, dsig, cfg.n_samples,
                                cfg.h_inv, d_o, d_d)
        elif getattr(sync, "per_plane", False):
            o = 0
            for i in range(3):
                ops.vm_scatter_rays(1, afs, gap, gal, comp.samp, b["aidx"], comp.sidx, b["a_count"], cap, dcomps,
                                    cfg.n_samples, cfg.h_inv, d_o, d_d, max_ctas=-80, plane_mask=1 << i)
                end = o + sizes[i] if i < 2 else n_app
                sync.on_app_grads(flat[o:end])
                o = end
            ops.vm_scatter_rays(0, dfs, gdp, gdl, comp.samp, None, comp.sidx, comp.count, cap_v, dsig, cfg.n_samples,
                                cfg.h_inv, d_o, d_d, max_ctas=-80)
            sync.on_rest(flat[n_app:])
        elif sync.use_split21(n_app, flat.numel()):
            ops.vm_scatter_rays(1, afs, gap, gal, comp.samp, b["aidx"], comp.sidx, b["a_count"], cap, dcomps,
                                cfg.n_samples, cfg.h_inv, d_o, d_d, plane_mask=3)
            n01 = sizes[0] + sizes[1]
            sync.on_app_grads(flat[:n01])
            ops.vm_scatter_rays(1, afs, gap, gal, comp.samp, b["aidx"], comp.sidx, b["a_count"], cap, dcomps,
                                cfg.n_samples, cfg.h_inv, d_o, d_d, max_ctas=-80, plane_mask=4)
            sync.on_app_grads(flat[n01:n_app])
            ops.vm_scatter_rays(0, dfs, gdp, gdl, comp.samp, None, comp.sidx, comp.count, cap_v, dsig, cfg.n_samples,
                                cfg.h_inv, d_o, d_d, max_ctas=-80)
            sync.on_rest(flat[n_app:])
        else:
            ops.vm_scatter_rays(1, afs, gap, gal, comp.samp, b["aidx"], comp.sidx, b["a_count"], cap, dcomps,
                                cfg.n_samples, cfg.h_inv, d_o, d_d)
            sync.on_app_grads(flat[:n_app])
            reserve = int(getattr(sync, "reserve_sms", 0))
            resident = 4 if dfs.C[0] == 16 else 3
            ops.vm_scatter_rays(0, dfs, gdp, gdl, comp.samp, None, comp.sidx, comp.count, cap_v, dsig, cfg.n_samples,
                                cfg.h_inv, d_o, d_d, max_ctas=((148 - reserve) * resident if reserve > 0 else -80))
            sync.on_rest(flat[n_app:])

        gdpn, gdln = FactorSet.grads_as_nchw(gdp, gdl)
        gapn, galn = FactorSet.grads_as_nchw(gap, gal)
        VMRender.last_grad_bucket = flat
        return (None, d_o, d_d, None, *gdpn, *gdln, *gapn, *galn, g_basis, *head_grads)


VMRender.last_grad_bucket = None
VMRender.debug_capture = None
VMRender.last_counts = None
```

Measured before the change: 1.487 million.

## Fold SH basis into per-ray matrices and skip dcomps materialization in scatter

```diff
diff --git a/include/jt_vm.h b/include/jt_vm.h
--- a/include/jt_vm.h
+++ b/include/jt_vm.h
@@ -37,6 +37,11 @@
                        const float* samp, const int* slot, const int* sidx, const int* n_dev, int n_max,
                        const void* gin, int gin_bf16, int n_samples, const float* h_inv, float* d_o, float* d_d,
                        int max_ctas, int plane_mask, cudaStream_t stream);
+int jt_sh_fold_rays(const float* rays_d, int n_rays, int normalize_dir, const float* Wb, void* mtab, cudaStream_t stream);
+int jt_vm_scatter_rays_sh(const void* const* h_factors, void* const* h_factor_grads, const int* h_dims,
+                          const float* samp, const int* slot, const int* sidx, const int* n_dev, int n_max,
+                          const float* dpre, const void* mtab, int n_samples, const float* h_inv, float* d_o, float* d_d,
+                          int max_ctas, int plane_mask, cudaStream_t stream);
 int jt_ray_init(const float* rays_d, const float* dnorm, int n_rays, float* d_o, float* d_d, cudaStream_t stream);
 
 int jt_gemm_nt(const float* X, int ldx, const float* W, int ldw, int w_kn, const float* bias, float* Y, int ldy,
diff --git a/joint-tensorf_b200/_lib.py b/joint-tensorf_b200/_lib.py
--- a/joint-tensorf_b200/_lib.py
+++ b/joint-tensorf_b200/_lib.py
@@ -13,6 +13,8 @@
     "jt_vm_gather_fwd": [_I, _P, _P, _P, _P, _P, _I, _P, _P],
     "jt_vm_gather_bwd": [_I, _P, _P, _P, _P, _P, _P, _I, _P, _P, _I, _P],
     "jt_vm_scatter_rays": [_I, _P, _P, _P, _P, _P, _P, _P, _I, _P, _I, _I, _P, _P, _P, _I, _I, _P],
+    "jt_sh_fold_rays": [_P, _I, _I, _P, _P, _P],
+    "jt_vm_scatter_rays_sh": [_P, _P, _P, _P, _P, _P, _P, _I, _P, _P, _I, _P, _P, _P, _I, _I, _P],
     "jt_ray_init": [_P, _P, _I, _P, _P, _P],
     "jt_gemm_nt": [_P, _I, _P, _I, _I, _P, _P, _I, _P, _I, _P, _I, _I, _I, _I, _P],
     "jt_gemm_tn": [_P, _I, _P, _I, _P, _I, _I, _I, _P, _I, _P, _P],
diff --git a/joint-tensorf_b200/csrc/shade_tc_bwd.cu b/joint-tensorf_b200/csrc/shade_tc_bwd.cu
--- a/joint-tensorf_b200/csrc/shade_tc_bwd.cu
+++ b/joint-tensorf_b200/csrc/shade_tc_bwd.cu
@@ -422,6 +422,46 @@
     tc_fence_before();
     __syncthreads();
     if (warp == 0) tmem_dealloc(tmem, 256);
+}
+
+__global__ void __launch_bounds__(NTB, 8) sh_bwd_df_kernel(const float* __restrict__ dout, const float* __restrict__ featdir,
+                                                           int ldf, const int* __restrict__ n_dev, int n_fixed,
+                                                           unsigned char* __restrict__ stage) {
+    __shared__ __align__(128) unsigned char dfs[2][SZ_DF];
+    const int tid = threadIdx.x;
+    const int r = tid & (TM - 1), hh = tid >> 7;
+    const int n = n_dev ? *n_dev : n_fixed;
+    int buf = 0;
+    for (int tile = blockIdx.x; (long long)tile * TM < n; tile += gridDim.x, buf ^= 1) {
+        const long long rw = (long long)tile * TM + r;
+        float4 g4 = make_float4(0.f, 0.f, 0.f, 0.f), d4 = g4;
+        if (rw < n) {
+            g4 = __ldg(reinterpret_cast<const float4*>(dout) + rw);
+            d4 = __ldcs(reinterpret_cast<const float4*>(featdir + (size_t)rw * ldf + 28));
+        }
+        const float d[3] = {d4.x, d4.y, d4.z};
+        const float go[3] = {g4.x, g4.y, g4.z};
+        float y[9], df[16];
+        sh9(d, y);
+#pragma unroll
+        for (int e = 0; e < 16; ++e) {
+            const int col = 16 * hh + e;
+            const int c0 = e / 9, k0 = e % 9, c1 = (16 + e) / 9, k1 = (16 + e) % 9;
+            const float v0 = go[c0] * y[k0];
+            const float v1 = (16 + e) < F_ ? go[c1 < 3 ? c1 : 0] * y[k1] : 0.f;
+            df[e] = col < F_ ? (hh == 0 ? v0 : v1) : 0.f;
+        }
+        store_chunk(dfs[buf], nullptr, TM, 2 * hh, r, df);
+        store_chunk(dfs[buf], nullptr, TM, 2 * hh + 1, r, df + 8);
+        fence_async_smem();
+        if (tid == 0) bulk_wait_read0();
+        __syncthreads();
+        if (tid == 0) {
+            bulk_s2g(stage + (size_t)tile * STAGE_TILE_BYTES + OFF_DF, dfs[buf], SZ_DF);
+            bulk_commit();
+        }
+    }
+    if (tid == 0) bulk_wait0();
 }
 
 }
@@ -460,8 +500,8 @@
 
 extern "C" int jt_sh_bwd_tc(const float* dout, const float* featdir, int ldf, const float* Wb, const int* n_dev,
                             int n_max, void* dcomps, int dcomps_bf16, void* stage, float* gWb, cudaStream_t stream) {
-    JT_CHECK_ARG(dout && featdir && Wb && dcomps && stage && gWb && ldf >= 32 && ldf % 4 == 0);
-    JT_CHECK_ARG(dcomps_bf16 == 1);
+    JT_CHECK_ARG(dout && featdir && Wb && stage && gWb && ldf >= 32 && ldf % 4 == 0);
+    JT_CHECK_ARG(!dcomps || dcomps_bf16 == 1);
     JT_CHECK_ARG((reinterpret_cast<uintptr_t>(stage) & 127) == 0 && (reinterpret_cast<uintptr_t>(dcomps) & 15) == 0);
     if (n_max <= 0) return JT_OK;
     long long tiles = ((long long)n_max + TM - 1) / TM;
@@ -471,8 +511,12 @@
     if (int rc = set_smem(head_bwd_wgrad_kernel<3, 1, WG_SH_STAGES, WG_SH_STAGE_BYTES>, WG_SH_STAGES * WG_SH_STAGE_BYTES)) return rc;
     g_launches += 2;
     unsigned char* st = static_cast<unsigned char*>(stage);
-    sh_bwd_data_kernel<<<grid_d, NTB, ShBwdSmem::total, stream>>>(dout, featdir, ldf, Wb, n_dev, n_max,
-                                                                 static_cast<unsigned short*>(dcomps), st);
+    if (dcomps)
+        sh_bwd_data_kernel<<<grid_d, NTB, ShBwdSmem::total, stream>>>(dout, featdir, ldf, Wb, n_dev, n_max,
+                                                                     static_cast<unsigned short*>(dcomps), st);
+    else
+        sh_bwd_df_kernel<<<(int)(tiles < 8 * kNumSMs ? tiles : 8 * kNumSMs), NTB, 0, stream>>>(dout, featdir, ldf, n_dev,
+                                                                                             n_max, st);
     head_bwd_wgrad_kernel<3, 1, WG_SH_STAGES, WG_SH_STAGE_BYTES><<<grid_w, TM, WG_SH_STAGES * WG_SH_STAGE_BYTES, stream>>>(
         st, n_dev, n_max, gWb, nullptr, nullptr, nullptr, nullptr, nullptr, nullptr);
     JT_RETURN_LAUNCH();
diff --git a/joint-tensorf_b200/csrc/vm_scatter.cu b/joint-tensorf_b200/csrc/vm_scatter.cu
--- a/joint-tensorf_b200/csrc/vm_scatter.cu
+++ b/joint-tensorf_b200/csrc/vm_scatter.cu
@@ -1,6 +1,7 @@
 #include <limits.h>
 #include <stdlib.h>
 #include <type_traits>
+#include <cuda_fp16.h>
 #include "jt_common.cuh"
 #include "../../include/jt_vm.h"
 
@@ -19,6 +20,14 @@
 __device__ __forceinline__ void f2_dot_acc(float2& acc, float4 a, float4 b) {
     acc = __ffma2_rn(lo2(a), lo2(b), acc);
     acc = __ffma2_rn(hi2(a), hi2(b), acc);
+}
+__device__ __forceinline__ uint2 f4_to_h4(float4 v) {
+    __half2 l = __floats2half2_rn(v.x, v.y), h = __floats2half2_rn(v.z, v.w);
+    return make_uint2(*reinterpret_cast<uint32_t*>(&l), *reinterpret_cast<uint32_t*>(&h));
+}
+__device__ __forceinline__ float4 h4_to_f4(uint2 u) {
+    const float2 l = __half22float2(*reinterpret_cast<const __half2*>(&u.x)), h = __half22float2(*reinterpret_cast<const __half2*>(&u.y));
+    return make_float4(l.x, l.y, h.x, h.y);
 }
 __device__ __forceinline__ bool f4_any(float4 a) { return a.x != 0.f || a.y != 0.f || a.z != 0.f || a.w != 0.f; }
 
@@ -50,6 +59,7 @@
     int seg;
     int seg_target;
     int plane_mask;
+    const uint4* mtab;
 };
 
 struct RaySums { float o[3], d[3]; };
@@ -73,10 +83,11 @@
     int sid;
 };
 
-template <bool APP, int NQ, int I, bool GB16, bool B16, int THR = SC_THREADS>
+template <bool APP, int NQ, int I, bool GB16, bool B16, bool SHF = false, int THR = SC_THREADS>
 __device__ __forceinline__ void walk_plane(const ScatterArgs& A, const int e0, const int e1, const int q, const int qs,
                                            int& ray, int& ray_end, RaySums& rs,
-                                           typename std::conditional<B16, uint2, float4>::type* __restrict__ sm) {
+                                           typename std::conditional<B16, uint2, float4>::type* __restrict__ sm,
+                                           float4* __restrict__ xs) {
     using SlotT = typename std::conditional<B16, uint2, float4>::type;
     using ElemT = typename std::conditional<B16, unsigned short, float>::type;
     const Factors& F = A.F;
@@ -141,7 +152,37 @@
             g[0].s = A.gin[e];
         }
     };
+    constexpr int MR = (SHF && !B16) ? 2 : 3;
+    static_assert(!SHF || NQ == 3, "SH shading: 3 x 48 components");
+    uint2 M[SHF ? MR : 1][NQ];
+    float msc = 1.f;
+    auto load_fold = [&](int r) {
+        const uint4* p = A.mtab + ((size_t)(r * 3 + I) * 4 + (q >> 2)) * 5;
+        const uint4 t0 = __ldg(p), t1 = __ldg(p + 1), t2 = __ldg(p + 2), t3 = __ldg(p + 3), t4 = __ldg(p + 4);
+        M[0][0] = make_uint2(t0.x, t0.y); M[0][1] = make_uint2(t0.z, t0.w); M[0][2] = make_uint2(t1.x, t1.y);
+        M[1][0] = make_uint2(t1.z, t1.w); M[1][1] = make_uint2(t2.x, t2.y); M[1][2] = make_uint2(t2.z, t2.w);
+        if constexpr (MR == 3) {
+            M[MR - 1][0] = make_uint2(t3.x, t3.y); M[MR - 1][1] = make_uint2(t3.z, t3.w); M[MR - 1][2] = make_uint2(t4.x, t4.y);
+        } else {
+            xs[2 * THR] = make_float4(__uint_as_float(t3.x), __uint_as_float(t3.y), __uint_as_float(t3.z), __uint_as_float(t3.w));
+            xs[3 * THR] = make_float4(__uint_as_float(t4.x), __uint_as_float(t4.y), 0.f, 0.f);
+        }
+        msc = __uint_as_float(t4.z);
+    };
+    auto dpre_copy = [&](int e) { cp_async16(xs + (e & 1) * THR, A.gin + 4 * (size_t)e); };
     auto gin_value = [&](const GinRaw g[NQ], int k) -> float4 {
+        if (SHF) {
+            float4 v = f4_scale(h4_to_f4(M[0][k]), dup2(g[0].f.x));
+            f4_fma(v, h4_to_f4(M[1][k]), dup2(g[0].f.y));
+            uint2 m2;
+            if constexpr (MR == 3) m2 = M[2 % MR][k];
+            else {
+                const float4 a = xs[(k == 2 ? 3 : 2) * THR];
+                m2 = k == 1 ? make_uint2(__float_as_uint(a.z), __float_as_uint(a.w)) : make_uint2(__float_as_uint(a.x), __float_as_uint(a.y));
+            }
+            f4_fma(v, h4_to_f4(m2), dup2(g[0].f.z));
+            return v;
+        }
         if (APP && GB16)
             return make_float4(__uint_as_float(g[k].h.x << 16), __uint_as_float(g[k].h.x & 0xFFFF0000u),
                                __uint_as_float(g[k].h.y << 16), __uint_as_float(g[k].h.y & 0xFFFF0000u));
@@ -177,6 +218,7 @@
         line_offs(pn.l0, oln);
         fetch_plane(0, on);
         fetch_line(0, oln);
+        if (SHF) dpre_copy(e0);
         cp_async_commit();
     }
     auto slot_of = [&](int e) -> int { return e < e1 ? (A.slot ? A.slot[e] : e) : 0; };
@@ -189,7 +231,8 @@
     }
     int jn2 = slot_of(e0 + 2);
     GinRaw gn[NQ];
-    load_gin(e0, gn);
+    if (SHF) load_fold(pn.sid / A.S);
+    else load_gin(e0, gn);
 
     for (int e = e0; e < e1; ++e) {
         const StepPos pc = pn;
@@ -210,7 +253,8 @@
                 lbn = lb ^ 1;
                 fetch_line(lbn, oln);
             }
-            load_gin(e + 1, gn);
+            if (SHF) dpre_copy(e + 1);
+            else load_gin(e + 1, gn);
             if (e + 2 < e1) {
                 un = A.samp[jn2];
                 sn = A.sidx[jn2];
@@ -224,6 +268,7 @@
             flush_ray();
             ray = pc.sid / A.S;
             ray_end = (ray + 1) * A.S;
+            if (SHF) load_fold(ray);
         }
         const int x0 = pc.x0, y0 = pc.y0, l0 = pc.l0;
         const float mx0 = (x0 >= 0 && x0 < W) ? 1.f : 0.f, mx1 = (x0 + 1 >= 0 && x0 + 1 < W) ? 1.f : 0.f;
@@ -256,6 +301,7 @@
         const float2 w00 = dup2(wx0 * wy0), w10 = dup2(wx1 * wy0), w01 = dup2(wx0 * wy1), w11 = dup2(wx1 * wy1);
         const float2 wl0p = dup2(wl0), wl1p = dup2(wl1);
         float2 dA2 = dup2(0.f), dB2 = dup2(0.f), dC2 = dup2(0.f), dD2 = dup2(0.f), dLa2 = dup2(0.f), dLb2 = dup2(0.f);
+        if (SHF) gc[0].f = f4_scale(xs[(e & 1) * THR], dup2(msc));
 #pragma unroll
         for (int k = 0; k < NQ; ++k) {
             const float4 a = rd(pslot(pb, 0, k)), b = rd(pslot(pb, 1, k)), c = rd(pslot(pb, 2, k)), d = rd(pslot(pb, 3, k));
@@ -296,7 +342,7 @@
     flush_ray();
 }
 
-template <bool APP, int NQ, int MINB, bool GB16, int LWC, bool B16>
+template <bool APP, int NQ, int MINB, bool GB16, int LWC, bool B16, bool SHF = false>
 __global__ void __launch_bounds__(SC_THREADS, MINB) vm_scatter_walk_kernel(const ScatterArgs A, int LW_rt, int walkers_per_cta) {
     extern __shared__ __align__(16) unsigned char sc_smem[];
     using SlotT = typename std::conditional<B16, uint2, float4>::type;
@@ -305,8 +351,9 @@
     const int wl = threadIdx.x / LW;
     const int q = (threadIdx.x - wl * LW) * 4;
     const int qs = LW * 4;
+    SlotT* sm = reinterpret_cast<SlotT*>(sc_smem) + threadIdx.x;
+    float4* xs = reinterpret_cast<float4*>(sc_smem + 12 * NQ * SC_THREADS * sizeof(SlotT)) + threadIdx.x;
     if (wl >= walkers_per_cta) return;
-    SlotT* sm = reinterpret_cast<SlotT*>(sc_smem) + threadIdx.x;
     const int stride = gridDim.x * walkers_per_cta;
     int seg = A.seg;
     if (A.seg_target > 0) {
@@ -322,20 +369,61 @@
         RaySums rs;
 #pragma unroll
         for (int a = 0; a < 3; ++a) rs.o[a] = rs.d[a] = 0.f;
-        if (A.plane_mask & 1) walk_plane<APP, NQ, 0, GB16, B16>(A, e0, e1, q, qs, ray, ray_end, rs, sm);
-        if (A.plane_mask & 2) walk_plane<APP, NQ, 1, GB16, B16>(A, e0, e1, q, qs, ray, ray_end, rs, sm);
-        if (A.plane_mask & 4) walk_plane<APP, NQ, 2, GB16, B16>(A, e0, e1, q, qs, ray, ray_end, rs, sm);
-    }
+        if (A.plane_mask & 1) walk_plane<APP, NQ, 0, GB16, B16, SHF>(A, e0, e1, q, qs, ray, ray_end, rs, sm, xs);
+        if (A.plane_mask & 2) walk_plane<APP, NQ, 1, GB16, B16, SHF>(A, e0, e1, q, qs, ray, ray_end, rs, sm, xs);
+        if (A.plane_mask & 4) walk_plane<APP, NQ, 2, GB16, B16, SHF>(A, e0, e1, q, qs, ray, ray_end, rs, sm, xs);
+    }
+}
+
+__global__ void sh_fold_kernel(const float* __restrict__ rays_d, int n_rays, int normalize_dir, const float* __restrict__ Wb,
+                               uint4* __restrict__ mtab) {
+    constexpr int CT = 144;
+    const int t = blockIdx.x * blockDim.x + threadIdx.x;
+    if (t >= n_rays * 12) return;
+    const int sub = t & 3, I = (t >> 2) % 3, ray = t / 12;
+    float d0 = rays_d[3 * ray], d1 = rays_d[3 * ray + 1], d2 = rays_d[3 * ray + 2];
+    if (normalize_dir) {
+        const float nn = sqrtf(d0 * d0 + d1 * d1 + d2 * d2);
+        d0 /= nn; d1 /= nn; d2 /= nn;
+    }
+    const float d[3] = {d0, d1, d2};
+    float y[9];
+    sh9(d, y);
+    float4 m[9];
+    float mx = 0.f;
+#pragma unroll
+    for (int ck = 0; ck < 9; ++ck) {
+        const int c = ck / 3, k = ck % 3;
+        float4 v = f4z();
+#pragma unroll
+        for (int kk = 0; kk < 9; ++kk) f4_fma(v, ldg4(Wb + (9 * c + kk) * CT + 48 * I + 16 * k + 4 * sub), dup2(y[kk]));
+        m[ck] = v;
+        mx = fmaxf(mx, fmaxf(fmaxf(fabsf(v.x), fabsf(v.y)), fmaxf(fabsf(v.z), fabsf(v.w))));
+    }
+    int ex;
+    frexpf(mx, &ex);
+    ex = mx > 0.f ? max(ex, -100) : 0;
+    const float2 up = dup2(ldexpf(1.f, 15 - ex));
+    uint2 h[9];
+#pragma unroll
+    for (int ck = 0; ck < 9; ++ck) h[ck] = f4_to_h4(f4_scale(m[ck], up));
+    uint4* o = mtab + (size_t)t * 5;
+    o[0] = make_uint4(h[0].x, h[0].y, h[1].x, h[1].y);
+    o[1] = make_uint4(h[2].x, h[2].y, h[3].x, h[3].y);
+    o[2] = make_uint4(h[4].x, h[4].y, h[5].x, h[5].y);
+    o[3] = make_uint4(h[6].x, h[6].y, h[7].x, h[7].y);
+    o[4] = make_uint4(h[8].x, h[8].y, __float_as_uint(ldexpf(1.f, ex - 15)), 0u);
 }
 
 }
 
 using namespace jt;
 
-extern "C" int jt_vm_scatter_rays(int app, const void* const* h_factors, void* const* h_factor_grads,
-                                  const int* h_dims, const float* samp, const int* slot, const int* sidx,
-                                  const int* n_dev, int n_max, const void* gin, int gin_bf16, int n_samples, const float* h_inv,
-                                  float* d_o, float* d_d, int max_ctas, int plane_mask, cudaStream_t stream) {
+static int scatter_launch(int app, const void* const* h_factors, void* const* h_factor_grads, const int* h_dims,
+                          const float* samp, const int* slot, const int* sidx, const int* n_dev, int n_max,
+                          const void* gin, int gin_bf16, const void* sh_mtab,
+                          int n_samples, const float* h_inv, float* d_o, float* d_d, int max_ctas, int plane_mask,
+                          cudaStream_t stream) {
     JT_CHECK_ARG(h_factors && h_factor_grads && h_dims && samp && sidx && gin && h_inv && d_o && d_d && n_samples > 0);
     JT_CHECK_ARG(plane_mask > 0 && plane_mask <= 7);
     if (n_max <= 0) return JT_OK;
@@ -353,6 +441,7 @@
     A.samp = reinterpret_cast<const float4*>(samp);
     A.slot = slot; A.sidx = sidx; A.n_dev = n_dev; A.n_fixed = n_max; A.gin = static_cast<const float*>(gin); A.gin_bf16 = gin_bf16;
     JT_CHECK_ARG(!gin_bf16 || app);
+    A.mtab = static_cast<const uint4*>(sh_mtab);
     A.d_o = d_o; A.d_d = d_d;
     for (int a = 0; a < 3; ++a) A.inv[a] = h_inv[a];
     A.S = n_samples;
@@ -364,6 +453,7 @@
     int nq = 1, LW = cmax / 4;
     const bool uniform = A.F.C[0] == A.F.C[1] && A.F.C[1] == A.F.C[2];
     if (uniform && (cmax == 48 || cmax == 32)) { nq = cmax / 16; LW = 4; }
+    if (sh_mtab && nq != 3) return JT_ERR_UNSUPPORTED;
     JT_CHECK_ARG(LW >= 1 && LW <= 128);
     const int wpc = SC_THREADS / LW;
     const int threads = ((wpc * LW + 31) / 32) * 32;
@@ -375,20 +465,48 @@
     if (A.seg_target > 0) want = cap;
     int grid = (int)(want < cap ? (want < 1 ? 1 : want) : cap);
     g_launches += 1;
-    const int smem = 12 * nq * SC_THREADS * (A.F.bf16 ? 8 : 16);
-#define JT_SCB(APPV, NQV, MB, GB, LWV, BV)                                                                          \
+    const int smem = 12 * nq * SC_THREADS * (A.F.bf16 ? 8 : 16) + (sh_mtab ? 4 * 16 * SC_THREADS : 0);
+#define JT_SCB(APPV, NQV, MB, GB, LWV, BV, SHV)                                                                     \
     {                                                                                                               \
         if (smem > 48 * 1024 &&                                                                                     \
-            cudaFuncSetAttribute(vm_scatter_walk_kernel<APPV, NQV, MB, GB, LWV, BV>,                                \
+            cudaFuncSetAttribute(vm_scatter_walk_kernel<APPV, NQV, MB, GB, LWV, BV, SHV>,                           \
                                  cudaFuncAttributeMaxDynamicSharedMemorySize, smem) != cudaSuccess)                 \
             return JT_ERR_LAUNCH;                                                                                   \
-        vm_scatter_walk_kernel<APPV, NQV, MB, GB, LWV, BV><<<grid, threads, smem, stream>>>(A, LW, wpc);            \
-    }
-#define JT_SC(APPV, NQV, MB, GB, LWV) { if (A.F.bf16) JT_SCB(APPV, NQV, MB, GB, LWV, true) else JT_SCB(APPV, NQV, MB, GB, LWV, false) }
-    if (app && gin_bf16) { if (nq == 3) JT_SC(true, 3, 2, true, 4) else if (nq == 2) JT_SC(true, 2, 3, true, 4) else JT_SC(true, 1, 3, true, 0) }
+        vm_scatter_walk_kernel<APPV, NQV, MB, GB, LWV, BV, SHV><<<grid, threads, smem, stream>>>(A, LW, wpc);       \
+    }
+#define JT_SC(APPV, NQV, MB, GB, LWV) { if (A.F.bf16) JT_SCB(APPV, NQV, MB, GB, LWV, true, false) else JT_SCB(APPV, NQV, MB, GB, LWV, false, false) }
+    if (sh_mtab) { if (A.F.bf16) JT_SCB(true, 3, 2, false, 4, true, true) else JT_SCB(true, 3, 2, false, 4, false, true) }
+    else if (app && gin_bf16) { if (nq == 3) JT_SC(true, 3, 2, true, 4) else if (nq == 2) JT_SC(true, 2, 3, true, 4) else JT_SC(true, 1, 3, true, 0) }
     else if (app) { if (nq == 3) JT_SC(true, 3, 2, false, 4) else if (nq == 2) JT_SC(true, 2, 3, false, 4) else JT_SC(true, 1, 3, false, 0) }
     else { if (nq == 3) JT_SC(false, 3, 2, false, 4) else if (nq == 2) JT_SC(false, 2, 3, false, 4) else JT_SC(false, 1, 4, false, 0) }
 #undef JT_SC
 #undef JT_SCB
     JT_RETURN_LAUNCH();
 }
+
+extern "C" int jt_vm_scatter_rays(int app, const void* const* h_factors, void* const* h_factor_grads,
+                                  const int* h_dims, const float* samp, const int* slot, const int* sidx,
+                                  const int* n_dev, int n_max, const void* gin, int gin_bf16, int n_samples, const float* h_inv,
+                                  float* d_o, float* d_d, int max_ctas, int plane_mask, cudaStream_t stream) {
+    return scatter_launch(app, h_factors, h_factor_grads, h_dims, samp, slot, sidx, n_dev, n_max, gin, gin_bf16, nullptr,
+                          n_samples, h_inv, d_o, d_d, max_ctas, plane_mask, stream);
+}
+
+extern "C" int jt_sh_fold_rays(const float* rays_d, int n_rays, int normalize_dir, const float* Wb, void* mtab,
+                               cudaStream_t stream) {
+    JT_CHECK_ARG(rays_d && Wb && mtab && n_rays >= 0 && (reinterpret_cast<uintptr_t>(mtab) & 15) == 0);
+    if (n_rays == 0) return JT_OK;
+    g_launches += 1;
+    const int threads = n_rays * 12;
+    sh_fold_kernel<<<(threads + 127) / 128, 128, 0, stream>>>(rays_d, n_rays, normalize_dir, Wb, static_cast<uint4*>(mtab));
+    JT_RETURN_LAUNCH();
+}
+
+extern "C" int jt_vm_scatter_rays_sh(const void* const* h_factors, void* const* h_factor_grads, const int* h_dims,
+                                     const float* samp, const int* slot, const int* sidx, const int* n_dev, int n_max,
+                                     const float* dpre, const void* mtab, int n_samples, const float* h_inv, float* d_o,
+                                     float* d_d, int max_ctas, int plane_mask, cudaStream_t stream) {
+    JT_CHECK_ARG(dpre && mtab);
+    return scatter_launch(1, h_factors, h_factor_grads, h_dims, samp, slot, sidx, n_dev, n_max, dpre, 0, mtab, n_samples,
+                          h_inv, d_o, d_d, max_ctas, plane_mask, stream);
+}
diff --git a/joint-tensorf_b200/ops.py b/joint-tensorf_b200/ops.py
--- a/joint-tensorf_b200/ops.py
+++ b/joint-tensorf_b200/ops.py
@@ -181,6 +181,25 @@
               "jt_vm_scatter_rays")
 
 
+def sh_fold_rays(rays_d, normalize_dir, wb):
+    n = int(rays_d.shape[0])
+    mtab = torch.empty((n * 960,), device=rays_d.device, dtype=torch.uint8)
+    with TIMER.span("sh_fold"):
+        check(_lib.lib().jt_sh_fold_rays(_p(rays_d), n, int(normalize_dir), _p(wb), _p(mtab), _stream()),
+              "jt_sh_fold_rays")
+    return mtab
+
+
+def vm_scatter_rays_sh(fs, gp, gl, samp, slot, sidx, n_dev, n_max, dpre, mtab, n_samples, h_inv, d_o, d_d,
+                       max_ctas=0, plane_mask=7):
+    gptrs = ptrs([g.data_ptr() for g in gp] + [g.data_ptr() for g in gl])
+    with TIMER.span("vm_app_bwd"):
+        check(_lib.lib().jt_vm_scatter_rays_sh(fs.ptrs, gptrs, fs.dims, _p(samp), _p(slot), _p(sidx), _p(n_dev),
+                                               int(n_max), _p(dpre), _p(mtab), int(n_samples), h_inv, _p(d_o),
+                                               _p(d_d), int(max_ctas), int(plane_mask), _stream()),
+              "jt_vm_scatter_rays_sh")
+
+
 def gemm_nt(x, ldx, w, ldw, w_kn, bias, y, ldy, mask, ldm, m_dev, m_max, n, k, act, name="gemm_nt",
             x_off=0, w_off=0, y_off=0, mask_off=0):
     with TIMER.span(name):
@@ -251,7 +270,8 @@
 def sh_bwd_tc(dout, featdir, wb, n_dev, n_max, dcomps, stage, g_basis):
     with TIMER.span("sh_bwd_tc"):
         check(_lib.lib().jt_sh_bwd_tc(_p(dout), _p(featdir), int(featdir.shape[1]), _p(wb), _p(n_dev), int(n_max),
-                                      _p(dcomps), int(dcomps.dtype == torch.bfloat16), _p(stage), _p(g_basis),
+                                      _p(dcomps), int(dcomps is not None and dcomps.dtype == torch.bfloat16),
+                                      _p(stage), _p(g_basis),
                                       _stream()), "jt_sh_bwd_tc")
 
 
diff --git a/joint-tensorf_b200/render.py b/joint-tensorf_b200/render.py
--- a/joint-tensorf_b200/render.py
+++ b/joint-tensorf_b200/render.py
@@ -294,13 +294,25 @@
             check(lib.jt_ray_init(_p(b["rays_d"]), _p(dnorm), N, _p(d_o), _p(d_d), _stream()), "jt_ray_init")
 
         wv_tc = cfg.head == "tc" and cfg.shading == "MLP_Fea_WeakView"
-        dcomps = torch.empty((cap, afs.ctot), device=dev,
-                             dtype=torch.bfloat16 if (cfg.head == "tc" and not wv_tc) else torch.float32)
+        sh_tc = cfg.head == "tc" and cfg.shading == "SH"
+        dcomps = None if sh_tc else torch.empty((cap, afs.ctot), device=dev,
+                                                dtype=torch.bfloat16 if (cfg.head == "tc" and not wv_tc) else torch.float32)
+
+        mtab = ops.sh_fold_rays(b["rays_d"], cfg.ndc, b["basis_w"]) if sh_tc else None
+
+        def app_scatter(**kw):
+            if sh_tc:
+                ops.vm_scatter_rays_sh(afs, gap, gal, comp.samp, b["aidx"], comp.sidx, b["a_count"], cap, dout, mtab,
+                                       cfg.n_samples, cfg.h_inv, d_o, d_d, **kw)
+            else:
+                ops.vm_scatter_rays(1, afs, gap, gal, comp.samp, b["aidx"], comp.sidx, b["a_count"], cap, dcomps,
+                                    cfg.n_samples, cfg.h_inv, d_o, d_d, **kw)
+
         if wv_tc:
             w1, b1, w2, b2, w3, b3 = b["head"]
             ops.wv_head_bwd_tc(dout, b["feat"], b["basis_w"], w1, w2, w3, b["a_count"], cap, cfg.fea_prog, dcomps,
                                ws["stage"], (g_basis, *head_grads))
-        elif cfg.head == "tc" and cfg.shading == "SH":
+        elif sh_tc:
             ops.sh_bwd_tc(dout, b["feat"], b["basis_w"], b["a_count"], cap, dcomps, ws["stage"], g_basis)
         elif cfg.head == "tc":
             w1, b1, w2, b2, w3, b3 = b["head"]
@@ -318,15 +330,13 @@
             ops.gemm_nt(dfeat, ldf, b["basis_w"], afs.ctot, 1, None, dcomps, afs.ctot, None, 0, b["a_count"], cap,
                         afs.ctot, F, 0, name="basis_bwd_x")
         if sync is None:
-            ops.vm_scatter_rays(1, afs, gap, gal, comp.samp, b["aidx"], comp.sidx, b["a_count"], cap, dcomps,
-                                cfg.n_samples, cfg.h_inv, d_o, d_d)
+            app_scatter()
             ops.vm_scatter_rays(0, dfs, gdp, gdl, comp.samp, None, comp.sidx, comp.count, cap_v, dsig, cfg.n_samples,
                                 cfg.h_inv, d_o, d_d)
         elif getattr(sync, "per_plane", False):
             o = 0
             for i in range(3):
-                ops.vm_scatter_rays(1, afs, gap, gal, comp.samp, b["aidx"], comp.sidx, b["a_count"], cap, dcomps,
-                                    cfg.n_samples, cfg.h_inv, d_o, d_d, max_ctas=-80, plane_mask=1 << i)
+                app_scatter(max_ctas=-80, plane_mask=1 << i)
                 end = o + sizes[i] if i < 2 else n_app
                 sync.on_app_grads(flat[o:end])
                 o = end
@@ -334,19 +344,16 @@
                                 cfg.h_inv, d_o, d_d, max_ctas=-80)
             sync.on_rest(flat[n_app:])
         elif sync.use_split21(n_app, flat.numel()):
-            ops.vm_scatter_rays(1, afs, gap, gal, comp.samp, b["aidx"], comp.sidx, b["a_count"], cap, dcomps,
-                                cfg.n_samples, cfg.h_inv, d_o, d_d, plane_mask=3)
+            app_scatter(plane_mask=3)
             n01 = sizes[0] + sizes[1]
             sync.on_app_grads(flat[:n01])
-            ops.vm_scatter_rays(1, afs, gap, gal, comp.samp, b["aidx"], comp.sidx, b["a_count"], cap, dcomps,
-                                cfg.n_samples, cfg.h_inv, d_o, d_d, max_ctas=-80, plane_mask=4)
+            app_scatter(max_ctas=-80, plane_mask=4)
             sync.on_app_grads(flat[n01:n_app])
             ops.vm_scatter_rays(0, dfs, gdp, gdl, comp.samp, None, comp.sidx, comp.count, cap_v, dsig, cfg.n_samples,
                                 cfg.h_inv, d_o, d_d, max_ctas=-80)
             sync.on_rest(flat[n_app:])
         else:
-            ops.vm_scatter_rays(1, afs, gap, gal, comp.samp, b["aidx"], comp.sidx, b["a_count"], cap, dcomps,
-                                cfg.n_samples, cfg.h_inv, d_o, d_d)
+            app_scatter()
             sync.on_app_grads(flat[:n_app])
             reserve = int(getattr(sync, "reserve_sms", 0))
             resident = 4 if dfs.C[0] == 16 else 3
```

After: 1.503 million (median of 6 runs). +1.0%, better.
